# rhasspy/larynx

Hardware: AMD Instinct MI355X
Metric: utterances_per_sec (higher is better)
Workload: dtype f32; 1 GPU; en-us ljspeech GlowTTS + hifi_gan 'high', batch=1, 120 phoneme ids per utterance (~623 frames = 7.24 s audio), seeded random weights, device RNG noise, fused one-call entry (mi355tts_synthesize), denoiser off (the Python API default); ids_per_utterance=120, parallelism=utterance-dp1, batch=1, calls_in_flight_per_gpu=8

## Files before the change

### include/mi355tts.h

```cpp
#ifndef MI355TTS_H
#define MI355TTS_H

#include <stddef.h>
#include <stdint.h>

#ifdef __cplusplus
extern "C" {
#endif

#define MI355TTS_ABI_VERSION 2

typedef enum {
  MI355TTS_OK = 0,
  MI355TTS_ERR_INVALID = -1,
  MI355TTS_ERR_HIP = -2,
  MI355TTS_ERR_NOMEM = -3,
  MI355TTS_ERR_TOO_SMALL = -4,
  MI355TTS_ERR_NO_MODEL = -5
} mi355tts_status;

typedef struct mi355tts_ctx mi355tts_ctx;
typedef struct mi355tts_mel mi355tts_mel;

typedef struct {
// ... 157 lines not shown
  int32_t sample_rate, hop, window, tau_min, tau_max;
  float threshold;
  int32_t interpolate;
} mi355tts_pitch_params;
int mi355tts_load_pitch(mi355tts_ctx* ctx, const mi355tts_pitch_params* params, int* model_out);
int64_t mi355tts_pitch_frames(mi355tts_ctx* ctx, int model, int64_t samples);
int mi355tts_pitch(mi355tts_ctx* ctx, int model, const float* in_f32, const int16_t* in_i16, const int64_t* samples, int B,
                   int64_t in_ld, float* f0_out, float* periodicity_out, float* level_db_out, float* cmnd_out, int64_t out_ld,
                   uint32_t flags);

typedef struct {
  int32_t up, down, window;
  int32_t pitch, resampler;
} mi355tts_shift_params;
int mi355tts_load_shift(mi355tts_ctx* ctx, const mi355tts_shift_params* params, const float* window, int* model_out);
int64_t mi355tts_shift_length(mi355tts_ctx* ctx, int model, int64_t samples);
int mi355tts_shift(mi355tts_ctx* ctx, int model, const float* in_f32, const int16_t* in_i16, const int64_t* samples, int B,
                   int64_t in_ld, const int32_t* positions_in, float* out_f32, int16_t* out_i16, int64_t out_ld, int pcm_mode,
                   int32_t* positions_out, int64_t pos_ld, float* f0_out, int64_t f0_ld, int64_t* samples_out, uint32_t flags);

int mi355tts_synthesize(mi355tts_ctx* ctx, int glow, int vocoder, const int64_t* ids, const int32_t* id_lens, int B,
                        int ids_ld, float noise_scale, float length_scale, const float* noise, int noise_ld, uint64_t seed,
                        const mi355tts_audio_settings* audio, float denoiser_strength, int32_t pad_before,
                        int32_t pad_after, int32_t* frames_out, float* wav_f32, int16_t* wav_i16, int64_t wav_ld,
                        uint32_t flags);

int mi355tts_synthesize_speakers(mi355tts_ctx* ctx, int glow, int vocoder, const int64_t* ids, const int32_t* id_lens, int B,
                                 int ids_ld, float noise_scale, float length_scale, const float* noise, int noise_ld,
                                 uint64_t seed, const int32_t* speaker_ids, const mi355tts_audio_settings* audio,
                                 float denoiser_strength, int32_t pad_before, int32_t pad_after, int32_t* frames_out,
                                 float* wav_f32, int16_t* wav_i16, int64_t wav_ld, uint32_t flags);

int mi355tts_synthesize_prosody(mi355tts_ctx* ctx, int glow, int vocoder, const int64_t* ids, const int32_t* id_lens, int B,
                                int ids_ld, float noise_scale, float length_scale, const float* noise, int noise_ld,
                                uint64_t seed, const int32_t* speaker_ids, const mi355tts_audio_settings* audio,
                                float denoiser_strength, int32_t pad_before, int32_t pad_after, int32_t* frames_out,
                                float* wav_f32, int16_t* wav_i16, int64_t wav_ld, uint32_t flags,
                                const mi355tts_prosody* prosody);

int mi355tts_reserve(mi355tts_ctx* ctx, int workers, int glow, int vocoder, int max_batch, int max_ids, int max_frames,
                     int denoiser, int max_pad_samples);
int mi355tts_worker_queue_groups(mi355tts_ctx* ctx, int32_t* groups, int capacity);

int mi355tts_op_conv1d(mi355tts_ctx* ctx, const float* x, int B, int Cin, int L, const int32_t* lens, const float* w,
                       const float* bias, int Cout, int K, int dilation, float in_slope, int out_act, float* y);
int mi355tts_op_conv_transpose1d(mi355tts_ctx* ctx, const float* x, int B, int Cin, int L, const float* w,
                                 const float* bias, int Cout, int K, int stride, float in_slope, float* y);

int mi355tts_op_denoise(mi355tts_ctx* ctx, const float* wav, int B, int64_t N, const float* bias_spec, float strength,
                        float* out);

int mi355tts_op_gauss_noise(mi355tts_ctx* ctx, uint64_t seed, int B, int C, int T, float* out);

int mi355tts_op_maximum_path(mi355tts_ctx* ctx, const float* value, int B, int P_ld, int F_ld, const int32_t* id_lens,
                             const int32_t* frames, int32_t* durations_out, int dur_ld, float* score_out);

int mi355tts_hifigan_infer_taps(mi355tts_ctx* ctx, int vocoder, const mi355tts_mel* mel, float* wav_f32, int64_t wav_ld, char* json,
                                int cap);
int mi355tts_voc_tap_copy(mi355tts_ctx* ctx, int index, float* dst, int64_t cap);

int mi355tts_bench_conv1d(mi355tts_ctx* ctx, int B, int Cin, int Cout, int K, int dilation, int L, int tile_shape,
                          int iters, float* ms_per_launch);

int mi355tts_set_profiling(mi355tts_ctx* ctx, int enabled);
int mi355tts_set_option(mi355tts_ctx* ctx, const char* name, int value);
int mi355tts_call_coalesce_default(void);
int mi355tts_coalesce_stats(mi355tts_ctx* ctx, int64_t* passes, int64_t* rows);
int mi355tts_dispatch_selfcheck(mi355tts_ctx* ctx, int* state, float* plain_us, float* snake_us);
int mi355tts_profile_reset(mi355tts_ctx* ctx);
int mi355tts_profile_json(mi355tts_ctx* ctx, char* buf, int cap);
int mi355tts_profile_kernels_json(mi355tts_ctx* ctx, char* buf, int cap);
int mi355tts_kernel_counts_json(mi355tts_ctx* ctx, char* buf, int cap);
int mi355tts_profile_event_overhead(mi355tts_ctx* ctx, int pairs, double* us_out);

#ifdef __cplusplus
}
#endif
#endif
```

### larynx_amd/csrc/conv_mfma.h

```cpp
#pragma once
#include <hip/hip_runtime.h>
#include "prio.h"
#include "tile_grid.h"

#ifdef MI355TTS_ABLATION
#define MI355TTS_ABLATE(a, bit) ((a).ablate & (bit))
#else
#define MI355TTS_ABLATE(a, bit) 0
#endif

#ifndef CONV_STAMP
#define CONV_STAMP(n)
#endif
#ifndef CONV_WG_STAMP
#define CONV_WG_STAMP(lin, which)
#endif
#ifndef CONV_CHUNK_STAMP
#define CONV_CHUNK_STAMP(chunk, which)
#endif
#ifndef MI355TTS_ARING
#define MI355TTS_ARING 3
#endif

namespace mi355tts {


typedef float floatx16 __attribute__((ext_vector_type(16)));

enum ConvEpilogue {
  EPI_LINEAR = 0,
  EPI_GATE = 1,
  EPI_COUPLING = 2,
  EPI_UPSAMPLE = 3,
};

enum OutAct { ACT_NONE = 0, ACT_RELU = 1, ACT_TANH = 2 };

struct ConvArgs {
  const float* x;
  const float* x2;
  const float* x3;
  float in_div;
  long long x_bs;
  int x_ld;
  const int* in_len;
  int in_mul;
  int in_const;
  const float* w;
  const float* bias;
  int noct;
  int Cin;
  int rows;
  int dil;
  int pad;
  float in_slope;
  float* y;
  long long y_bs;
  int y_ld;
  const float* res;
  float* y2;
  long long y2_bs;
  int y2_ld;
  int split;
  int accum;
  int accum2;
  float alpha;
  int out_act;
  const int* out_len;
  int out_mul;
  int out_const;
  int up;
  int up_pad;
  int half;
  const float* cond;
  long long cond_bs;
  float* mix_x0;
  const float* mix_w;
  const float* mix_bias;
  const float* mix_scale;
  int ablate;
  int rows_major;
  const void* w16;
  int nslab;
};

template <int K, int EPI>
__device__ __forceinline__ int conv_n_len(const ConvArgs& a, int b) {
  if constexpr (EPI == EPI_UPSAMPLE) {
    const int Lin = a.in_len ? a.in_len[b] * a.in_mul : a.in_const;
    return Lin > 0 ? Lin + (K - 1) : 0;
  } else {
    return a.out_len ? a.out_len[b] * a.out_mul : a.out_const;
  }
}

template <int K, int CI_C, int MB, int NB, int WN, int KS, int HALO, int EPI, int WM = 1>
constexpr int conv_lds_floats() {
  constexpr bool SCATTER = (EPI == EPI_LINEAR || EPI == EPI_GATE);
  constexpr int NBR = (SCATTER && NB > 2) ? 1 : NB;
  constexpr int RED = (KS - 1) * WM * WN * NBR * 16 * 64;
  constexpr int XS = 2 * CI_C * (WN * NB * 32 + HALO);
  return XS > RED ? XS : RED;
}

template <int K, int CI_C, int MB, int NB, int WN, int KS, int HALO, int EPI, int WM = 1>
__device__ __forceinline__ void conv_tile(const ConvArgs& a, const int tile_x, const int tile_y, const int b, float* __restrict__ xs) {
  static_assert(WM == 1 || EPI == EPI_LINEAR || EPI == EPI_UPSAMPLE, "row groups of waves: linear and upsample epilogues");
  constexpr int NWAVES = WM * WN * KS;
  constexpr int WX = WM * WN;
  constexpr int NT = 64 * NWAVES;
  constexpr int T_T = WN * NB * 32;
  constexpr int XW = T_T + HALO;
  constexpr int OCTS = CI_C / 8;
  constexpr int NO = OCTS / KS;
  constexpr int S = NO * K;
  constexpr bool SCATTER = (EPI == EPI_LINEAR || EPI == EPI_GATE);
  constexpr int NBR = (SCATTER && NB > 2) ? 1 : NB;
  constexpr int RED = (KS - 1) * WX * NBR * 16 * 64;
  constexpr int LDSF = conv_lds_floats<K, CI_C, MB, NB, WN, KS, HALO, EPI, WM>();
  static_assert(CI_C % 8 == 0 && CI_C % NWAVES == 0 && OCTS % KS == 0, "bad tile parameters");

  const int tid = threadIdx.x;
  const int lane = tid & 63;
  const int wave = tid >> 6;
  const int wm = wave % WM;
  const int wn = (wave / WM) % WN;
  const int kg = wave / WX;
  const int wx = wm * WN + wn;
  const int t0 = tile_x * T_T;
  const int mt0 = (tile_y * WM + wm) * MB;

  const int Lin = a.in_len ? a.in_len[b] * a.in_mul : a.in_const;
  const int Lout = a.out_len ? a.out_len[b] * a.out_mul : a.out_const;
  const int n_len = (EPI == EPI_UPSAMPLE) ? (Lin > 0 ? Lin + (K - 1) : 0) : Lout;
  if (t0 >= n_len) return;

  const int roww = T_T + (K - 1) * a.dil;
  const float slope = a.in_slope;
  const float* xb = a.x + (long long)b * a.x_bs;
  const float* xb2 = a.x2 ? a.x2 + (long long)b * a.x_bs : nullptr;
  const float* xb3 = a.x3 ? a.x3 + (long long)b * a.x_bs : nullptr;
  const int nchunks = ((a.Cin + 7) / 8 + OCTS - 1) / OCTS;

  constexpr int XW4 = XW / 4;
  constexpr int NF4 = CI_C * XW4;
  constexpr int NE = (NF4 + NT - 1) / NT;
  static_assert(XW % 4 == 0, "LDS row stride must be a multiple of 4 floats");
  constexpr bool PD1 = (WN == 1 && KS == 8 && MB == 2 && K >= 7);
  float4 preA[NE], preB[PD1 ? 1 : NE];
  const int PA = (a.pad + 3) & ~3;
  const int used4 = (PA - a.pad + roww + 3) >> 2;
  const int cin_last = a.Cin - 1;
  const int ld_last4 = a.x_ld - 4;
  auto gload = [&](int chunk, float4 (&pre)[NE]) {
    int off[NE];
#pragma unroll
    for (int i = 0; i < NE; ++i) {
      const int e = tid + NT * i;
      const int row = e / XW4, f = e - row * XW4;
      const int ci = chunk * CI_C + (row < CI_C ? row : CI_C - 1);
      const int c0 = t0 - PA + 4 * f;
      off[i] = (ci < a.Cin ? ci : cin_last) * a.x_ld + (c0 < 0 ? 0 : (c0 > ld_last4 ? ld_last4 : c0));
    }
#pragma unroll
    for (int i = 0; i < NE; ++i) pre[i] = *reinterpret_cast<const float4*>(xb + off[i]);
#ifndef MI355TTS_PROBE_NO_X2
    if (xb2) {
      float4 t2[NE];
#pragma unroll
      for (int i = 0; i < NE; ++i) t2[i] = *reinterpret_cast<const float4*>(xb2 + off[i]);
#pragma unroll
      for (int i = 0; i < NE; ++i) {
        pre[i].x += t2[i].x;
        pre[i].y += t2[i].y;
        pre[i].z += t2[i].z;
        pre[i].w += t2[i].w;
      }
      if (xb3) {
#pragma unroll
        for (int i = 0; i < NE; ++i) t2[i] = *reinterpret_cast<const float4*>(xb3 + off[i]);
#pragma unroll
        for (int i = 0; i < NE; ++i) {
          pre[i].x += t2[i].x;
          pre[i].y += t2[i].y;
          pre[i].z += t2[i].z;
          pre[i].w += t2[i].w;
        }
      }
#pragma unroll
      for (int i = 0; i < NE; ++i) {
        pre[i].x = pre[i].x / a.in_div;
        pre[i].y = pre[i].y / a.in_div;
        pre[i].z = pre[i].z / a.in_div;
        pre[i].w = pre[i].w / a.in_div;
      }
    }
#endif
  };
  auto lstore = [&](int buf, int chunk, const float4 (&pre)[NE]) {
    float4* dst = reinterpret_cast<float4*>(xs + buf * (CI_C * XW));
#pragma unroll
    for (int i = 0; i < NE; ++i) {
      const int e = tid + NT * i;
      const int row = e / XW4, f = e - row * XW4;
      const int c0 = t0 - PA + 4 * f;
      const bool fok = chunk * CI_C + row < a.Cin && f < used4;
      float4 v = pre[i];
      v.x = (fok && c0 >= 0 && c0 < Lin) ? v.x : 0.f;
      v.y = (fok && c0 + 1 >= 0 && c0 + 1 < Lin) ? v.y : 0.f;
      v.z = (fok && c0 + 2 >= 0 && c0 + 2 < Lin) ? v.z : 0.f;
      v.w = (fok && c0 + 3 >= 0 && c0 + 3 < Lin) ? v.w : 0.f;
      v.x = v.x > 0.f ? v.x : v.x * slope;
      v.y = v.y > 0.f ? v.y : v.y * slope;
      v.z = v.z > 0.f ? v.z : v.z * slope;
      v.w = v.w > 0.f ? v.w : v.w * slope;
      if (e < NF4) dst[e] = v;
    }
  };

  floatx16 acc[MB][NB];
#pragma unroll
  for (int mb = 0; mb < MB; ++mb)
#pragma unroll
    for (int nb = 0; nb < NB; ++nb)
#pragma unroll
      for (int r = 0; r < 16; ++r) acc[mb][nb][r] = 0.f;

  const float4* wq[MB];
#pragma unroll
  for (int mb = 0; mb < MB; ++mb)
    wq[mb] = reinterpret_cast<const float4*>(a.w) + (long long)(mt0 + mb) * a.noct * K * 64 + lane;
  const int last_chunk = nchunks - 1;
  const int last_step = nchunks * S - 1;
  auto a_index = [&](int chunk, int q) -> long long {
    int g = chunk * S + q;
    g = g < last_step ? g : last_step;
    const int ch = g / S;
    q = g - ch * S;
    const int oi = q / K;
    const int k = q - oi * K;
    return (long long)(((ch * OCTS + kg + oi * KS) * K + k)) * 64;
  };

  constexpr int RD = MI355TTS_ARING;
  float4 ar[RD][MB];

  CONV_STAMP(0);
// ... 142 lines not shown
#pragma unroll
              for (int rr = 0; rr < R; ++rr)
                own[mb][nb0 + nbi][rr] += red[((((kg * (KS - 1) + si) * WX + wx) * NBR + nbi) * R + rr) * 64 + lane];
        }
    }
  } else if constexpr (KS > 1) {
    float* red = xs;
#pragma unroll
    for (int mb = 0; mb < MB; ++mb) {
      if (mb > 0) __syncthreads();
      if (kg > 0) {
#pragma unroll
        for (int nb = 0; nb < NB; ++nb)
#pragma unroll
          for (int r = 0; r < 16; ++r)
            red[((((kg - 1) * WX + wx) * NB + nb) * 16 + r) * 64 + lane] = acc[mb][nb][r];
      }
      __syncthreads();
      if (kg == 0) {
#pragma unroll
        for (int g = 1; g < KS; ++g)
#pragma unroll
          for (int nb = 0; nb < NB; ++nb)
#pragma unroll
            for (int r = 0; r < 16; ++r)
              acc[mb][nb][r] += red[((((g - 1) * WX + wx) * NB + nb) * 16 + r) * 64 + lane];
      }
    }
    if (kg > 0) return;
  }

  CONV_STAMP(4);
  const int col = lane & 31;
  const int rbase = 4 * (lane >> 5);

  if constexpr (EPI == EPI_LINEAR) {
    int rowin[R];
#pragma unroll
    for (int rr = 0; rr < R; ++rr) {
      const int r = kg * R + rr;
      rowin[rr] = acc_row(r) + rbase;
    }
#pragma unroll
    for (int mb = 0; mb < MB; ++mb) {
      const int row0 = (mt0 + mb) * 32;
      const bool first = row0 < a.split;
      float* yp = first ? a.y : a.y2;
      const long long ybs = first ? a.y_bs : a.y2_bs;
      const int yld = first ? a.y_ld : a.y2_ld;
      const int rowoff = first ? 0 : a.split;
      const float* rp = first ? a.res : nullptr;
      const bool acc_on = first ? (a.accum != 0) : (a.accum2 != 0);
      const float alpha = first ? a.alpha : 1.0f;
      const int act = first ? a.out_act : (int)ACT_NONE;
      float bb[R];
      int roff[R];
      bool rok[R];
#pragma unroll
      for (int rr = 0; rr < R; ++rr) {
        const int row = row0 + rowin[rr];
        bb[rr] = a.bias ? a.bias[row] : 0.f;
        rok[rr] = row < a.rows;
        roff[rr] = ((rok[rr] ? row : a.rows - 1) - rowoff) * yld;
      }
      float v[NB][R];
      int tcol[NB];
      bool tok[NB];
#pragma unroll
      for (int nb = 0; nb < NB; ++nb) {
        const int t = t0 + (wn * NB + nb) * 32 + col;
        tok[nb] = t < Lout;
        tcol[nb] = tok[nb] ? t : Lout - 1;
#pragma unroll
        for (int rr = 0; rr < R; ++rr) v[nb][rr] = own[mb][nb][rr] + bb[rr];
      }
      float* yb = yp + (long long)b * ybs;
      if (rp) {
        const float* rb = rp + (long long)b * ybs;
        float rv[NB][R];
#pragma unroll
        for (int nb = 0; nb < NB; ++nb)
#pragma unroll
          for (int rr = 0; rr < R; ++rr) rv[nb][rr] = rb[roff[rr] + tcol[nb]];
#pragma unroll
        for (int nb = 0; nb < NB; ++nb)
#pragma unroll
          for (int rr = 0; rr < R; ++rr) v[nb][rr] += rv[nb][rr];
      }
#pragma unroll
      for (int nb = 0; nb < NB; ++nb)
#pragma unroll
        for (int rr = 0; rr < R; ++rr) v[nb][rr] *= alpha;
      if (acc_on) {
        float ov[NB][R];
#pragma unroll
        for (int nb = 0; nb < NB; ++nb)
#pragma unroll
          for (int rr = 0; rr < R; ++rr) ov[nb][rr] = yb[roff[rr] + tcol[nb]];
#pragma unroll
        for (int nb = 0; nb < NB; ++nb)
#pragma unroll
          for (int rr = 0; rr < R; ++rr) v[nb][rr] += ov[nb][rr];
      }
      if (act == ACT_RELU) {
#pragma unroll
        for (int nb = 0; nb < NB; ++nb)
#pragma unroll
          for (int rr = 0; rr < R; ++rr) v[nb][rr] = v[nb][rr] > 0.f ? v[nb][rr] : 0.f;
      } else if (act == ACT_TANH) {
#pragma unroll
        for (int nb = 0; nb < NB; ++nb)
#pragma unroll
          for (int rr = 0; rr < R; ++rr) v[nb][rr] = tanhf(v[nb][rr]);
      }
#pragma unroll
      for (int nb = 0; nb < NB; ++nb)
#pragma unroll
        for (int rr = 0; rr < R; ++rr)
          if (rok[rr] && tok[nb]) yb[roff[rr] + tcol[nb]] = v[nb][rr];
    }
  } else if constexpr (EPI == EPI_GATE) {
    static_assert(MB == 1, "paired epilogues use one 32-row tile: 16 rows of each half");
    constexpr int H = R / 2;
    static_assert(H >= 1, "GATE needs at most 8 k-groups");
    float b0[H], b1[H];
    int off[H];
    bool cok[H];
#pragma unroll
    for (int rr = 0; rr < H; ++rr) {
      const int r = kg * H + rr;
      const int i = acc_row(r) + rbase;
      b0[rr] = a.bias ? a.bias[mt0 * 32 + i] : 0.f;
      b1[rr] = a.bias ? a.bias[mt0 * 32 + 16 + i] : 0.f;
      const int c = tile_y * 16 + i;
      cok[rr] = c < a.half;
      if (a.cond) {
        const float* cd = a.cond + (long long)b * a.cond_bs + (cok[rr] ? c : a.half - 1);
        b0[rr] += cd[0];
        b1[rr] += cd[a.half];
      }
      off[rr] = (cok[rr] ? c : a.half - 1) * a.y_ld;
    }
#pragma unroll
    for (int nb = 0; nb < NB; ++nb) {
      const int t = t0 + (wn * NB + nb) * 32 + col;
      const bool tok = t < Lout;
      float* yb = a.y + (long long)b * a.y_bs + (tok ? t : Lout - 1);
#pragma unroll
      for (int rr = 0; rr < H; ++rr) {
        const float v0 = own[0][nb][rr] + b0[rr];
        const float v1 = own[0][nb][H + rr] + b1[rr];
        const float out = tanhf(v0) * (1.0f / (1.0f + expf(-v1)));
        if (cok[rr] && tok) yb[off[rr]] = out;
      }
    }
  } else if constexpr (EPI == EPI_COUPLING) {
    static_assert(MB == 1, "paired epilogues use one 32-row tile: 16 rows of each half");
    float b0[8], b1[8];
#pragma unroll
    for (int r = 0; r < 8; ++r) {
      const int i = (r & 3) + 8 * (r >> 2) + rbase;
      b0[r] = a.bias ? a.bias[mt0 * 32 + i] : 0.f;
      b1[r] = a.bias ? a.bias[mt0 * 32 + 16 + i] : 0.f;
    }
#pragma unroll
    for (int nb = 0; nb < NB; ++nb) {
// ... 73 lines not shown
            const int row0 = (mt0 + mb) * 32 + 8 * g4 + rbase;
            if (row0 >= a.rows) continue;
            const int co = row0 / a.up;
            const int n0 = q * a.up + (row0 - co * a.up) - a.up_pad;
            float* dst = a.y + (long long)b * a.y_bs + (long long)co * a.y_ld + n0;
            if (n0 >= 0 && n0 + 3 < Lout) {
              *reinterpret_cast<float4*>(dst) = make_float4(acc[mb][nb][4 * g4] + bb[4 * g4], acc[mb][nb][4 * g4 + 1] + bb[4 * g4 + 1],
                                                            acc[mb][nb][4 * g4 + 2] + bb[4 * g4 + 2], acc[mb][nb][4 * g4 + 3] + bb[4 * g4 + 3]);
            } else {
#pragma unroll
              for (int e = 0; e < 4; ++e)
                if (n0 + e >= 0 && n0 + e < Lout) dst[e] = acc[mb][nb][4 * g4 + e] + bb[4 * g4 + e];
            }
          }
          continue;
        }
#ifndef MI355TTS_NO_UP2_PAIR
        if (a.up == 2) {
#pragma unroll
          for (int r = 0; r < 16; r += 2) {
            const int row = (mt0 + mb) * 32 + (r & 3) + 8 * (r >> 2) + rbase;
            if (row >= a.rows) continue;
            const int co = row >> 1;
            const int n0 = q * 2 - a.up_pad;
            float* dst = a.y + (long long)b * a.y_bs + (long long)co * a.y_ld + n0;
            const float v0 = acc[mb][nb][r] + bb[r], v1 = acc[mb][nb][r + 1] + bb[r + 1];
            if (n0 >= 0 && n0 + 1 < Lout && row + 1 < a.rows) {
              typedef float up_float2 __attribute__((ext_vector_type(2), aligned(4)));
              *reinterpret_cast<up_float2*>(dst) = up_float2{v0, v1};
            } else {
              if (n0 >= 0 && n0 < Lout) dst[0] = v0;
              if (row + 1 < a.rows && n0 + 1 >= 0 && n0 + 1 < Lout) dst[1] = v1;
            }
          }
          continue;
        }
#endif
#pragma unroll
        for (int r = 0; r < 16; ++r) {
          const int row = (mt0 + mb) * 32 + (r & 3) + 8 * (r >> 2) + rbase;
          if (row >= a.rows) continue;
          const int co = row / a.up;
          const int ph = row - co * a.up;
          const int n = q * a.up + ph - a.up_pad;
          if (n < 0 || n >= Lout) continue;
          a.y[(long long)b * a.y_bs + (long long)co * a.y_ld + n] = acc[mb][nb][r] + bb[r];
        }
      }
    }
  }
}


template <int K, int CI_C, int MB, int NB, int WN, int KS, int HALO, int EPI, int WM = 1>
__global__ __launch_bounds__(64 * WM * WN * KS, ((EPI == EPI_LINEAR && ((NB == 1 && MB == 2) || (MB == 1 && NB == 2 && KS == 4))) || WM == 4) ? 4 : 1) void conv_mfma_kernel(const ConvArgs a) {
  __shared__ float xs[conv_lds_floats<K, CI_C, MB, NB, WN, KS, HALO, EPI, WM>()];
  int tile_x, tile_y;
  int gx = gridDim.x;
  const int lin = blockIdx.x + blockIdx.y * gridDim.x;
  if (gridDim.z > 1) {
    gx = row_tiles(conv_n_len<K, EPI>(a, blockIdx.z), WN * NB * 32);
    if (lin >= gx * (int)gridDim.y) return;
  }
  xcd_tile_lin(lin, gx, gridDim.y, tile_x, tile_y, a.rows_major);
  conv_tile<K, CI_C, MB, NB, WN, KS, HALO, EPI, WM>(a, tile_x, tile_y, blockIdx.z, xs);
  CONV_STAMP(5);
}

constexpr int GROUP_MAX_SEG = 8;
struct ConvGroupArgs {
  ConvArgs c[3];
  int gx[3], gy[3];
  int off[4];
  int nseg = 0;
  int seg_off[GROUP_MAX_SEG + 1];
  int seg_first[GROUP_MAX_SEG];
  int seg_m[GROUP_MAX_SEG];
};

inline void group_snake_order(ConvGroupArgs& g, int ncu, int slots) {
  g.nseg = 0;
  const int total = g.off[3];
  if (ncu <= 0 || (ncu & 7) || total <= ncu || total > slots) return;
  struct Piece { int m, first, n; };
  Piece out[GROUP_MAX_SEG];
  int nout = 0;
  for (int r0 = 0; r0 < total; r0 += ncu) {
    const int r1 = r0 + ncu < total ? r0 + ncu : total;
    Piece round[3];
    int nr = 0;
    for (int m = 0; m < 3; ++m) {
      const int a = g.off[m] > r0 ? g.off[m] : r0, b = g.off[m + 1] < r1 ? g.off[m + 1] : r1;
      if (b > a) round[nr++] = Piece{m, a - g.off[m], b - a};
    }
    const bool rev = ((r0 / ncu) & 1) != 0;
    for (int i = 0; i < nr; ++i) {
      const Piece& pc = round[rev ? nr - 1 - i : i];
      if (nout && out[nout - 1].m == pc.m && out[nout - 1].first + out[nout - 1].n == pc.first) {
        out[nout - 1].n += pc.n;
        continue;
      }
      if (nout == GROUP_MAX_SEG) return;
      out[nout++] = pc;
    }
  }
  int o = 0;
  for (int i = 0; i < nout; ++i) {
    g.seg_off[i] = o;
    g.seg_first[i] = out[i].first;
    g.seg_m[i] = out[i].m;
    o += out[i].n;
  }
  g.seg_off[nout] = o;
  g.nseg = nout;
}

inline double group_order_imbalance(const ConvGroupArgs& g, int ncu, const int real[3], const double cost[3]) {
  if (ncu <= 0 || ncu > 4096) return 1e9;
// ... 54 lines not shown
```

### larynx_amd/csrc/hifigan_forward.h

```cpp
#pragma once

extern "C" int mi355tts_hifigan_hop(mi355tts_ctx* ctx, int vocoder) {
  if (!ctx) return fail(MI355TTS_ERR_INVALID, "ctx null");
  std::shared_ptr<HifiModel> vpin;
  CHECK(find_model(ctx, vocoder, &vpin));
  return vpin->hop;
}

struct VocCall {
  float denoiser_strength = 0.f;
  float* wav_f32 = nullptr;
  int16_t* wav_i16 = nullptr;
  int64_t wav_ld = 0;
  uint32_t flags = 0;
  int pad_before = 0, pad_after = 0;
  const VocRow* rows = nullptr;
  int precision = -1;
  VocTaps* taps = nullptr;
};

static int ensure_denoiser_bias(mi355tts_ctx* ctx, HifiModel* hm, int vocoder, int precision);

static int hifigan_precheck(mi355tts_ctx* ctx, HifiModel* hm, int vocoder, const int32_t* frames, int B, int M, int Fmax, VocCall& c) {
  if (c.precision < 0) c.precision = hm->precision.load();
// ... 90 lines not shown
  VocTaps* taps;

  VocPass(CallFrame& f, HifiModel* hm_, const mi355tts_mel* mel_, const VocCall& call)
      : frame(f), ctx(f.ctx), w(f.w), hm(hm_), mel(mel_), s(f.s), B(mel_->B), F(mel_->max_frames), hop(hm_->hop), d_frames(mel_->frames_dev),
        voc_host_len(mel_->B == 1 ? mel_->frames[0] : -1), opt(f.w->opt), prec(call.precision), f16(call.precision == MI355TTS_PRECISION_F16),
        denoiser_strength(call.denoiser_strength), denoise(call.denoiser_strength > 0.f && mel_->max_frames > 0),
        out_dev((call.flags & MI355TTS_OUT_DEVICE) != 0), taps(call.taps) {}

  RowLen rows(int mul) const { return row_len(B, voc_host_len, d_frames, mul); }
  template <class P>
  P* plane(int i) const { return reinterpret_cast<P*>(buf[i]); }

  int bind(const VocCall& call, const OutRows& out) {
    const mi355tts_hifigan_hparams& h = hm->hp;
    if (f16 && !hm->f16_ok) return fail(MI355TTS_ERR_INVALID, "internal: fp16 mode on a vocoder it does not cover");
    bias_spec = hm->bias_spec[f16 ? 1 : 0];
    if (denoise && !bias_spec) return fail(MI355TTS_ERR_INVALID, "internal: no denoiser bias for this precision");
    voc_out = f16 || (!opt.env.voc_out_off && opt.voc_out && hm->post_C == (h.upsample_initial_channel >> h.num_upsamples) && hm->post.K == 7);
    if (call.rows && !voc_out) return fail(MI355TTS_ERR_INVALID, "internal: per-row outputs need the voc_out tail");
    for (int b = 0; b < B; ++b) {
      const OutRow r = out(b);
      pads = std::max(pads, (int)(r.pad_before + r.pad_after));
      any_f32 = any_f32 || r.f32;
      any_i16 = any_i16 || r.i16;
    }
    const HifiLayout lay = hifi_layout(h, hop, B, F, denoise, f16 || hifi_split_out(opt.serial_branches, h), pads);
    if (f16 && (size_t)((mel->M + 7) / 8) * F * 16 > lay.plane * sizeof(float)) return fail(MI355TTS_ERR_INVALID, "internal: mel octets exceed a plane buffer");
    staged = host_staging(B, any_f32 && !out_dev, (size_t)F * hop, any_i16 && !out_dev, (size_t)F * hop + (size_t)pads);
    CHECK(frame.reserve(lay.total, staged.end()));
    char* base = w->arena;
    for (int i = 0; i < lay.nbuf; ++i) buf[i] = (float*)(base + lay.o_buf[i]);
    wav = (float*)(base + lay.o_wav);
    wav2 = (float*)(base + lay.o_wav2);
    fbuf = (float*)(base + lay.o_fbuf);
    i16 = (short*)(base + lay.o_i16);
    peaks = (unsigned*)(base + lay.o_peak);
    Nld = lay.Nld;
    ild = Nld + (size_t)pads;
    Tmax = lay.Tmax;
    peak_ld = (long long)(Nld / POST_TW + 2);
    peak = voc_out && any_i16 && !denoise ? reinterpret_cast<float*>(peaks) : nullptr;
    return 0;
  }
};

static std::string tap_name(const char* fmt, ...) {
  char tmp[64];
  va_list ap;
  va_start(ap, fmt);
  std::vsnprintf(tmp, sizeof(tmp), fmt, ap);
  va_end(ap);
  return tmp;
}
static int voc_tap(VocPass& p, const std::string& name, const void* x, bool f16, int ch, int ld, int mul) {
  VocTaps& T = *p.taps;
  VocTap t;
  t.name = name;
  t.kn = T.last_kn;
  t.f16 = f16;
  t.B = p.B;
  t.ch = ch;
  t.ld = ld;
  for (int b = 0; b < p.B; ++b) t.len.push_back((int)std::min<long long>((long long)p.mel->frames[b] * mul, ld));
  t.bytes = f16 ? (size_t)p.B * (size_t)((ch + 7) / 8) * (size_t)ld * 16 : sizeof(float) * (size_t)p.B * (size_t)ch * (size_t)ld;
  if (T.bytes + t.bytes > VocTaps::MAX_BYTES)
    return fail(MI355TTS_ERR_NOMEM, "the planes of this call exceed %zu MB of tap copies (at '%s'): fewer frames or rows", VocTaps::MAX_BYTES >> 20, name.c_str());
  HIPCHECK(hipMalloc(&t.dev, t.bytes));
  T.bytes += t.bytes;
  T.taps.push_back(t);
  HIPCHECK(hipMemcpyAsync(t.dev, x, t.bytes, hipMemcpyDeviceToDevice, p.s));
  return 0;
}

struct VocStage {
  int i, u, ku, cout, Lout, ldo, mul;
  long long bs;
};
static VocStage voc_stage(const mi355tts_hifigan_hparams& h, int i, int Lin, int mul, bool f16) {
  VocStage st;
  st.i = i;
  st.u = h.upsample_rates[i];
  st.ku = h.upsample_kernel_sizes[i];
  st.cout = h.upsample_initial_channel >> (i + 1);
  st.Lout = Lin * st.u;
  st.ldo = f16 ? st.Lout : (st.Lout + 3) & ~3;
  st.mul = mul * st.u;
  st.bs = f16 ? (long long)(st.cout / 8) * st.ldo : (long long)st.cout * st.ldo;
  return st;
}

template <class P>
struct StageCursor {
  P* cur[3] = {nullptr, nullptr, nullptr};
  int ncur = 1;
  float div = 1.0f;
  int ch = 0, Lin = 0, ldin = 0, mul = 1;
  int flip = 0;

  template <class Args>
  void inputs(Args& a) const {
    a.x = cur[0];
    if (ncur > 1) {
      a.x2 = cur[1];
      a.x3 = ncur > 2 ? cur[2] : nullptr;
      a.in_div = div;
    }
  }
  void advance(const VocStage& st, P* const* outs, int n, float d, bool flipped) {
    for (int j = 0; j < 3; ++j) cur[j] = j < n ? outs[j] : nullptr;
    ncur = n;
    div = d;
    ch = st.cout;
// ... 24 lines not shown
  if (n_side > 0) {
    HIPCHECK(hipEventRecord(w->ev_fork, s));
    for (int j = 0; j < n_side; ++j) HIPCHECK(hipStreamWaitEvent(w->aux[j], w->ev_fork, 0));
  }
  CHECK(body());
  for (int j = 0; j < n_side; ++j) {
    HIPCHECK(hipEventRecord(w->ev_join[j], w->aux[j]));
    HIPCHECK(hipStreamWaitEvent(s, w->ev_join[j], 0));
  }
  return 0;
}

struct F32Schedule {
  bool split_out, grouped, concurrent;
  int rb_tiles;
};
static int f32_schedule(const VocPass& p, F32Schedule& sc) {
  const mi355tts_hifigan_hparams& h = p.hm->hp;
  const CallOptions& opt = p.opt;
  Worker* w = p.w;
  sc.split_out = hifi_split_out(opt.serial_branches, h);
  const bool busy = opt.adaptive_schedule && p.ctx->active_calls.load(std::memory_order_relaxed) > 1;
  sc.grouped = sc.split_out && h.num_kernels == 3 && opt.mrf_group && !busy;
  sc.concurrent = sc.split_out && !opt.mrf_group && !busy;
  if (p.taps && sc.concurrent)
    return fail(MI355TTS_ERR_INVALID, "taps: the forked schedule (\"mrf_group\" = 0) runs its chains on side streams a copy cannot be ordered behind");
  if (sc.concurrent && !w->aux[0]) {
    for (int i = 0; i < 2; ++i) {
      HIPCHECK(hipStreamCreateWithFlags(&w->aux[i], hipStreamNonBlocking));
      HIPCHECK(hipEventCreateWithFlags(&w->ev_join[i], hipEventDisableTiming));
    }
    HIPCHECK(hipEventCreateWithFlags(&w->ev_fork, hipEventDisableTiming));
  }
  sc.rb_tiles = opt.env.rb_tiles > 0 ? opt.env.rb_tiles : 1024;
  return 0;
}

static int f32_pre(VocPass& p, StageCursor<float>& c) {
  const int C0 = p.hm->hp.upsample_initial_channel, Fp = (p.F + 3) & ~3;
  c.cur[0] = p.buf[0];
  c.ch = C0;
  c.Lin = p.F;
  c.ldin = Fp;
  ConvArgs a = base_args(p.mel->voc, (long long)p.mel->M * p.mel->ld, p.mel->ld, p.d_frames, 1, c.cur[0], (long long)C0 * Fp, Fp, p.d_frames, 1, 1, 3);
  if (p.taps) CHECK(voc_tap(p, "mel", p.mel->voc, false, p.mel->M, p.mel->ld, 1));
  CHECK(launch_conv(p.ctx, p.w, p.hm->pre, a, EPI_LINEAR, p.B, p.F, KC_VOC_IO, nullptr, 1024, p.voc_host_len));
  if (p.taps) CHECK(voc_tap(p, "pre", c.cur[0], false, C0, Fp, 1));
  return 0;
}

static int f32_upsample(VocPass& p, const StageCursor<float>& c, const VocStage& st) {
  ConvArgs a = base_args(c.cur[0], (long long)c.ch * c.ldin, c.ldin, p.d_frames, c.mul, p.buf[1], st.bs, st.ldo, p.d_frames, st.mul, 1, st.ku / st.u - 1);
  c.inputs(a);
  a.in_slope = 0.1f;
  a.up = st.u;
  a.up_pad = (st.ku - st.u) / 2;
  CHECK(launch_conv(p.ctx, p.w, p.hm->ups[st.i], a, EPI_UPSAMPLE, p.B, c.Lin + st.ku / st.u - 1, KC_UPSAMPLE, nullptr, 1024, p.voc_host_len, p.prec));
  if (p.taps) CHECK(voc_tap(p, tap_name("up%d", st.i), p.buf[1], false, st.cout, st.ldo, st.mul));
  return 0;
}

struct VocStep {
  PairPlan pair;
  ConvPlan c1, c2;
  float* dst;
};
static int run_step_grouped(mi355tts_ctx* ctx, Worker* w, const VocStep (&sp)[3], hipStream_t s) {
  const int npair = sp[0].pair.ok + sp[1].pair.ok + sp[2].pair.ok;
  if (npair == 3) {
    const PairPlan* pairs[3] = {&sp[0].pair, &sp[1].pair, &sp[2].pair};
    return run_pair_group(ctx, w, pairs, 3, s);
  }
  if (npair != 0) return 1;
  const ConvPlan* c1[3] = {&sp[0].c1, &sp[1].c1, &sp[2].c1};
  const ConvPlan* c2[3] = {&sp[0].c2, &sp[1].c2, &sp[2].c2};
  const int rc = run_group(ctx, w, c1, 3, s);
  if (rc != 0 || sp[0].c2.empty) return rc;
  const int rc2 = run_group(ctx, w, c2, 3, s);
  if (rc2 == 1)
    for (int j = 0; j < 3; ++j) CHECK(run_plan(ctx, w, sp[j].c2, s));
  return rc2 < 0 ? rc2 : 0;
}

struct F32Chains {
  VocPass& p;
  const F32Schedule& sc;
  const VocStage& st;
  int nk, nd;
  ChainPlanes<float> pl[MI355TTS_MAX_STAGES];
  const float* rin[MI355TTS_MAX_STAGES];
  hipStream_t stream[MI355TTS_MAX_STAGES];

  F32Chains(VocPass& p_, const F32Schedule& sc_, const VocStage& st_, int flip)
      : p(p_), sc(sc_), st(st_), nk(p_.hm->hp.num_kernels), nd(p_.hm->hp.num_dilations) {
    for (int j = 0; j < nk; ++j) {
      pl[j] = chain_planes<float>(p, j, flip, sc.split_out);
      rin[j] = p.buf[1];
      stream[j] = (sc.concurrent && j > 0) ? p.w->aux[j - 1] : p.s;
    }
  }

  int plan_step(int j, int d, VocStep& sp) const {
    const mi355tts_hifigan_hparams& h = p.hm->hp;
    const HifiResConv& rc = p.hm->rb[st.i][j][d];
    const int kk = h.resblock_kernel_sizes[j], B = p.B, ldo = st.ldo, mul = st.mul, Lout = st.Lout, host_len = p.voc_host_len;
    const long long bs = st.bs;
    const int* d_frames = p.d_frames;
    const float* x = rin[j];
    const float inv_nk = 1.0f / (float)nk;
    sp.dst = step_dst(pl[j], d, nd);
    if (!sp.dst) return fail(MI355TTS_ERR_INVALID, "internal: resblock scratch aliasing");
    const bool fold = d == nd - 1 && !sc.split_out;
    sp.pair.ok = false;
    if (h.resblock_type == 1) {
      plan_pair(p.opt, rc.c1, rc.c2, x, sp.dst, bs, ldo, d_frames, mul, rc.dil, fold ? inv_nk : 1.0f, fold ? (j > 0) : 0, B, Lout, host_len,
                &sp.pair, p.prec);
      if (sp.pair.ok) return 0;
      ConvArgs a = base_args(x, bs, ldo, d_frames, mul, pl[j].t, bs, ldo, d_frames, mul, rc.dil, (kk * rc.dil - rc.dil) / 2);
      a.in_slope = 0.1f;
      CHECK(plan_conv(p.opt, rc.c1, a, EPI_LINEAR, B, Lout, KC_RESBLOCK, sc.rb_tiles, host_len, &sp.c1, p.prec));
      ConvArgs c2 = base_args(pl[j].t, bs, ldo, d_frames, mul, sp.dst, bs, ldo, d_frames, mul, 1, (kk - 1) / 2);
      c2.in_slope = 0.1f;
      c2.res = x;
      if (fold) {
        c2.alpha = inv_nk;
        c2.accum = j > 0;
      }
      CHECK(plan_conv(p.opt, rc.c2, c2, EPI_LINEAR, B, Lout, KC_RESBLOCK, sc.rb_tiles, host_len, &sp.c2, p.prec));
    } else {
      ConvArgs a = base_args(x, bs, ldo, d_frames, mul, sp.dst, bs, ldo, d_frames, mul, rc.dil, (kk * rc.dil - rc.dil) / 2);
      a.in_slope = 0.1f;
      a.res = x;
      if (fold) {
        a.alpha = inv_nk;
        a.accum = j > 0;
      }
      CHECK(plan_conv(p.opt, rc.c1, a, EPI_LINEAR, B, Lout, KC_RESBLOCK, sc.rb_tiles, host_len, &sp.c1, p.prec));
      sp.c2.empty = true;
    }
    return 0;
  }
  int tap_step(int j, int d, const VocStep& sp) const {
    const bool fold = d == nd - 1 && !sc.split_out;
    if (!sp.pair.ok && !sp.c2.empty) CHECK(voc_tap(p, tap_name("rb%d.%d.%d.t", st.i, j, d), pl[j].t, false, st.cout, st.ldo, st.mul));
    if (!fold) return voc_tap(p, tap_name("rb%d.%d.%d", st.i, j, d), sp.dst, false, st.cout, st.ldo, st.mul);
    return j == nk - 1 ? voc_tap(p, tap_name("stage%d", st.i), sp.dst, false, st.cout, st.ldo, st.mul) : 0;
  }
  int run_step_alone(int j, const VocStep& sp) const {
    if (sp.pair.ok) return run_pair(p.ctx, p.w, sp.pair, stream[j]);
    CHECK(run_plan(p.ctx, p.w, sp.c1, stream[j]));
    return run_plan(p.ctx, p.w, sp.c2, stream[j]);
  }
  int run_dilation_major() {
    for (int d = 0; d < nd; ++d) {
      VocStep sp[3];
      for (int j = 0; j < nk; ++j) CHECK(plan_step(j, d, sp[j]));
      if (nk == 3 && !sp[0].pair.ok && !sp[1].pair.ok && !sp[2].pair.ok) {
        ConvPlan* c1s[3] = {&sp[0].c1, &sp[1].c1, &sp[2].c1};
        ConvPlan* c2s[3] = {&sp[0].c2, &sp[1].c2, &sp[2].c2};
        promote_group_plans(p.opt, c1s, nk);
        promote_group_plans(p.opt, c2s, nk);
      }
      const int rc = sc.grouped ? run_step_grouped(p.ctx, p.w, sp, p.s) : 1;
      if (rc < 0) return rc;
      if (rc == 1)
        for (int j = 0; j < nk; ++j) CHECK(run_step_alone(j, sp[j]));
      if (p.taps)
        for (int j = 0; j < nk; ++j) CHECK(tap_step(j, d, sp[j]));
      for (int j = 0; j < nk; ++j) rin[j] = sp[j].dst;
    }
    return 0;
  }
  int run_chain_major() {
    for (int j = 0; j < nk; ++j)
      for (int d = 0; d < nd; ++d) {
        VocStep sp;
        CHECK(plan_step(j, d, sp));
        CHECK(run_step_alone(j, sp));
        if (p.taps) CHECK(tap_step(j, d, sp));
        rin[j] = sp.dst;
      }
    return 0;
  }
};

static int f32_resblocks(VocPass& p, const F32Schedule& sc, StageCursor<float>& c, const VocStage& st) {
  HifiModel* hm = p.hm;
  const int nk = hm->hp.num_kernels;
  if (p.opt.mrf_small && !p.opt.serial_branches && st.i < (int)hm->mrf.size() && hm->mrf[st.i].ok) {
    float* sums[2] = {p.buf[0], p.buf[2]};
    CHECK(run_mrf_small(p.ctx, p.w, hm->mrf[st.i], hm->arena, p.buf[1], sums[0], sums[1], st.bs, st.ldo, p.d_frames, st.mul, p.B, st.Lout, p.voc_host_len, p.s));
    if (p.taps)
      for (int m = 0; m < 2; ++m) CHECK(voc_tap(p, tap_name("stage%d.sum%d", st.i, m), sums[m], false, st.cout, st.ldo, st.mul));
    c.advance(st, sums, 2, (float)nk, false);
    return 0;
  }
  F32Chains chains(p, sc, st, c.flip);
  CHECK(run_forked(p.w, p.s, sc.concurrent ? nk - 1 : 0, [&] { return sc.split_out ? chains.run_dilation_major() : chains.run_chain_major(); }));
  if (sc.split_out) {
    float* outs[3] = {nullptr, nullptr, nullptr};
    for (int j = 0; j < nk; ++j) outs[j] = chains.pl[j].dst_last;
    c.advance(st, outs, nk, (float)nk, true);
  } else {
    std::swap(p.buf[5], p.buf[0]);
    c.advance(st, &p.buf[0], 1, 1.0f, false);
  }
  return 0;
}

template <class Args, class P>
static Args post_args(const VocPass& p, const StageCursor<P>& c, long long x_bs) {
  Args a;
  std::memset(&a, 0, sizeof(a));
  a.in_div = 1.0f;
  c.inputs(a);
  a.slope = 0.01f;
  a.x_bs = x_bs;
  a.x_ld = c.ldin;
  p.rows(c.mul).into(a);
  a.len_mul = c.mul;
  a.w = p.hm->arena + p.hm->post_w_off;
  a.bias = p.hm->arena + p.hm->post_b_off;
  a.C = c.ch;
  a.y = p.wav;
  a.y_bs = (long long)p.Nld;
  return a;
}

static int f32_post(VocPass& p, const StageCursor<float>& c) {
  if (!p.voc_out) {
    ConvArgs a = base_args(c.cur[0], (long long)c.ch * c.ldin, c.ldin, p.d_frames, c.mul, p.wav, (long long)p.Nld, (int)p.Nld, p.d_frames, c.mul, 1, 3);
    c.inputs(a);
    a.in_slope = 0.01f;
    a.out_act = ACT_TANH;
    CHECK(launch_conv(p.ctx, p.w, p.hm->post, a, EPI_LINEAR, p.B, c.Lin, KC_VOC_IO, nullptr, 1024, p.voc_host_len));
    if (p.taps) CHECK(voc_tap(p, "wav", p.wav, false, 1, (int)p.Nld, c.mul));
    return 0;
  }
  PostArgs a = post_args<PostArgs>(p, c, (long long)c.ch * c.ldin);
  if (p.peak) {
    a.peak = p.peak;
    a.peak_ld = p.peak_ld;
  }
  {
    ProfScope ps(p.ctx, p.w, KC_VOC_IO, 2.0 * (double)c.ch * 7 * (double)c.Lin * p.B);
    ps.kernel(KN_POST_CONV);
    const dim3 pg((c.Lin + POST_TW - 1) / POST_TW, p.B);
    switch_const<1, 2, 3>(c.ncur, [&](auto n) { hipLaunchKernelGGL(HIP_KERNEL_NAME(post_conv_kernel<7, decltype(n)::value>), pg, dim3(256), 0, p.s, a); });
  }
  if (p.taps) CHECK(voc_tap(p, "wav", p.wav, false, 1, (int)p.Nld, c.mul));
  return 0;
}

static int hifigan_body_f32(VocPass& p) {
  F32Schedule sc;
  CHECK(f32_schedule(p, sc));
  StageCursor<float> c;
  CHECK(f32_pre(p, c));
  for (int i = 0; i < p.hm->hp.num_upsamples; ++i) {
    const VocStage st = voc_stage(p.hm->hp, i, c.Lin, c.mul, false);
    CHECK(f32_upsample(p, c, st));
    CHECK(f32_resblocks(p, sc, c, st));
  }
  return f32_post(p, c);
}

struct HPlane {
  uint4* x;
  int ch, ld, mul;
};
static HConvArgs f16_conv_args(const VocPass& p, const HPlane& in, const HPlane& out, int dil, int pad) {
  HConvArgs a;
  std::memset(&a, 0, sizeof(a));
  a.x = in.x;
  a.x_bs = (long long)(in.ch / 8) * in.ld;
  a.x_ld = in.ld;
  a.in_div = 1.0f;
  a.dil = dil;
  a.pad = pad;
  a.in_slope = 1.0f;
  a.out_slope = 1.0f;
  a.y = out.x;
  a.y_bs = (long long)(out.ch / 8) * out.ld;
  a.y_ld = out.ld;
  a.cout = out.ch;
  h_set_lengths(a, p.B, p.d_frames, p.voc_host_len, in.mul, out.mul);
  return a;
}

static int f16_pre(VocPass& p, StageCursor<uint4>& c) {
  const mi355tts_mel* mel = p.mel;
  const int B = p.B, F = p.F, M = mel->M, moct = (M + 7) / 8, C0 = p.hm->hp.upsample_initial_channel;
  uint4* melh = p.plane<uint4>(1);
  {
    ProfScope ps(p.ctx, p.w, KC_SMALL, 0, p.s);
    ps.kernel(KN_PACK_OCTETS);
    hipLaunchKernelGGL(pack_octets_kernel, dim3((F + 255) / 256, moct, B), dim3(256), 0, p.s, mel->voc, (long long)mel->M * mel->ld, mel->ld, M, p.d_frames, 1,
                       melh, (long long)moct * F, F);
  }
  if (p.taps) CHECK(voc_tap(p, "mel", melh, true, 8 * moct, F, 1));
  c.cur[0] = p.plane<uint4>(0);
// ... 43 lines not shown
static int f16_resblocks(VocPass& p, StageCursor<uint4>& c, const VocStage& st) {
  const mi355tts_hifigan_hparams& h = p.hm->hp;
  const int nk = h.num_kernels, nd = h.num_dilations, B = p.B, ch = st.cout, Lout = st.Lout;
  ChainPlanes<uint4> pl[3];
  uint4* rin[3];
  auto plane = [&](uint4* x) { return HPlane{x, ch, st.ldo, st.mul}; };
  for (int j = 0; j < nk; ++j) {
    pl[j] = chain_planes<uint4>(p, j, c.flip, true);
    rin[j] = p.plane<uint4>(1);
  }
  const bool use_group = p.opt.mrf_group, use_pair = h.resblock_type == 1 && use_group && p.opt.rb_pair;
  for (int d = 0; d < nd; ++d) {
    HPlan c1[3], c2[3];
    HPairPlan pp[3];
    uint4* dst[3];
    for (int j = 0; j < nk; ++j) {
      const HResConv& rc = p.hm->h_rb[st.i][j][d];
      const int K = h.resblock_kernel_sizes[j], dil = h.resblock_dilations[j][d];
      const double flop = 2.0 * ch * ch * K * (double)Lout * B;
      dst[j] = step_dst(pl[j], d, nd);
      if (h.resblock_type == 1) {
        HConvArgs a1 = f16_conv_args(p, plane(rin[j]), plane(pl[j].t), dil, (K * dil - dil) / 2);
        HConvArgs a2 = f16_conv_args(p, plane(pl[j].t), plane(dst[j]), 1, (K - 1) / 2);
        a1.in_slope = a1.out_slope = 0.1f;
        a2.res = rin[j];
        c1[j] = plan_f16(rc.c1, a1, EPI_LINEAR, B, Lout, flop);
        c2[j] = plan_f16(rc.c2, a2, EPI_LINEAR, B, Lout, flop);
        pp[j].a = f16_pair_args(p, st, rc, rin[j], dst[j], dil);
        pp[j].K = K;
        pp[j].flop = 2.0 * flop;
      } else {
        HConvArgs a = f16_conv_args(p, plane(rin[j]), plane(dst[j]), dil, (K * dil - dil) / 2);
        a.in_slope = 0.1f;
        a.res = rin[j];
        c1[j] = plan_f16(rc.c1, a, EPI_LINEAR, B, Lout, flop);
      }
    }
    int fused = 1;
    if (use_pair) {
      fused = run_pair_group_f16(p.ctx, p.w, pp, nk, ch, B, Lout, p.s);
      if (fused < 0) return fused;
      if (fused == 0 && p.taps)
        for (int j = 0; j < nk; ++j) CHECK(voc_tap(p, tap_name("rb%d.%d.%d", st.i, j, d), dst[j], true, ch, st.ldo, st.mul));
    }
    for (int pass = 0; fused != 0 && pass < (h.resblock_type == 1 ? 2 : 1); ++pass) {
      const HPlan* plans = pass ? c2 : c1;
      int rc = use_group ? run_group_f16(p.ctx, p.w, plans, nk, B, p.s) : 1;
      if (rc < 0) return rc;
      if (rc == 1)
        for (int j = 0; j < nk; ++j) CHECK(run_plan_f16(p.ctx, p.w, plans[j], KC_RESBLOCK, p.s));
      if (p.taps) {
        const bool t_plane = h.resblock_type == 1 && pass == 0;
        for (int j = 0; j < nk; ++j)
          CHECK(voc_tap(p, tap_name(t_plane ? "rb%d.%d.%d.t" : "rb%d.%d.%d", st.i, j, d), t_plane ? pl[j].t : dst[j], true, ch, st.ldo, st.mul));
      }
    }
    for (int j = 0; j < nk; ++j) rin[j] = dst[j];
  }
  uint4* outs[3] = {nullptr, nullptr, nullptr};
  for (int j = 0; j < nk; ++j) outs[j] = pl[j].dst_last;
  c.advance(st, outs, nk, (float)nk, true);
  return 0;
}

static int f16_post(VocPass& p, const StageCursor<uint4>& c) {
  HPostArgs a = post_args<HPostArgs>(p, c, (long long)(c.ch / 8) * c.ldin);
  a.peak = p.peak;
  a.peak_ld = p.peak_ld;
  {
    ProfScope ps(p.ctx, p.w, KC_VOC_IO, 2.0 * (double)c.ch * 7 * (double)c.Lin * p.B, p.s);
    ps.kernel(KN_POST_F16);
    const dim3 pg((c.Lin + HPOST_TW - 1) / HPOST_TW, p.B);
    switch_const<1, 2, 3>(c.ncur, [&](auto n) { hipLaunchKernelGGL(HIP_KERNEL_NAME(post_f16_kernel<7, decltype(n)::value>), pg, dim3(256), 0, p.s, a); });
  }
  if (p.taps) CHECK(voc_tap(p, "wav", p.wav, false, 1, (int)p.Nld, c.mul));
  return 0;
}

static int hifigan_body_f16(VocPass& p) {
  StageCursor<uint4> c;
  CHECK(f16_pre(p, c));
  for (int i = 0; i < p.hm->hp.num_upsamples; ++i) {
    const VocStage st = voc_stage(p.hm->hp, i, c.Lin, c.mul, true);
    CHECK(f16_upsample(p, c, st));
    CHECK(f16_resblocks(p, c, st));
  }
  return f16_post(p, c);
}

static float* voc_denoise(VocPass& p) {
  if (!p.denoise) return p.wav;
  ProfScope ps(p.ctx, p.w, KC_SMALL, 0);
  hipLaunchKernelGGL(stft_denoise_kernel, dim3(p.Tmax, p.B), dim3(256), 0, p.s, p.wav, (long long)p.Nld, p.d_frames, p.hop, p.bias_spec,
                     p.denoiser_strength, p.fbuf, p.Tmax, (float*)nullptr);
  hipLaunchKernelGGL(overlap_add_kernel, dim3(256, p.B), dim3(256), 0, p.s, p.fbuf, p.Tmax, p.d_frames, p.hop, p.wav2, (long long)p.Nld,
                     (long long)p.Nld);
  return p.wav2;
}

static int voc_tail_one_launch(VocPass& p, const VocCall& call, float* wav) {
  const bool out_dev = p.out_dev;
  const int B = p.B;
  ProfScope ps(p.ctx, p.w, KC_SMALL, 0);
  if (p.any_i16 && !p.peak) {
    HIPCHECK(hipMemsetAsync(p.peaks, 0, sizeof(unsigned) * B, p.s));
    hipLaunchKernelGGL(absmax_kernel, dim3(128, B), dim3(256), 0, p.s, wav, (long long)p.Nld, p.d_frames, p.hop, p.peaks);
  }
// ... 105 lines not shown
    c.flags = MI355TTS_OUT_DEVICE;
    c.precision = precision;
    rc = hifigan_call_on(ctx, hm, vocoder, zm, c);
  }
  if (!rc) {
    CallFrame f(ctx);
    rc = f.open();
    if (!rc) {
      hipLaunchKernelGGL(stft_denoise_kernel, dim3(1, 1), dim3(256), 0, f.s, dwav, (long long)N, zm->frames_dev, hop,
                         (const float*)nullptr, 0.f, (float*)nullptr, 1, bias);
      if (f.wait() != hipSuccess) rc = fail(MI355TTS_ERR_HIP, "denoiser bias kernel failed");
    }
  }
  mel_destroy(zm);
  if (dwav) hipFree(dwav);
  if (rc) {
    if (bias) hipFree(bias);
    return rc;
  }
  hm->bias_spec[bi] = bias;
  hm->bias_ready[bi] = true;
  return 0;
}

static int hifigan_call(mi355tts_ctx* ctx, int vocoder, const mi355tts_mel* mel, const VocCall& call) {
  if (!ctx || !mel) return fail(MI355TTS_ERR_INVALID, "null argument");
  std::shared_ptr<HifiModel> vpin;
  CHECK(find_model(ctx, vocoder, &vpin));
  return hifigan_call_on(ctx, vpin.get(), vocoder, mel, call);
}

extern "C" int mi355tts_hifigan_infer_padded(mi355tts_ctx* ctx, int vocoder, const mi355tts_mel* mel, float denoiser_strength,
                                             float* wav_f32, int16_t* wav_i16, int64_t wav_ld, uint32_t flags,
                                             int32_t pad_before, int32_t pad_after) {
  VocCall c;
  c.denoiser_strength = denoiser_strength;
  c.wav_f32 = wav_f32;
  c.wav_i16 = wav_i16;
  c.wav_ld = wav_ld;
  c.flags = flags;
  c.pad_before = pad_before;
  c.pad_after = pad_after;
  return hifigan_call(ctx, vocoder, mel, c);
}

static std::string voc_taps_json(const VocTaps& T) {
  std::string s = "[";
  for (size_t i = 0; i < T.taps.size(); ++i) {
    const VocTap& t = T.taps[i];
    char tmp[256];
    std::snprintf(tmp, sizeof(tmp), "%s{\"name\": \"%s\", \"channels\": %d, \"ld\": %d, \"len\": [", i ? ", " : "", t.name.c_str(), t.ch, t.ld);
    s += tmp;
    for (size_t b = 0; b < t.len.size(); ++b) s += (b ? ", " : "") + std::to_string(t.len[b]);
    std::snprintf(tmp, sizeof(tmp), "], \"f16\": %d, \"kernel\": \"%s\"}", t.f16 ? 1 : 0, t.kn >= 0 && t.kn < KN_COUNT ? kname_name[t.kn] : "-");
    s += tmp;
  }
  return s + "]";
}

extern "C" int mi355tts_hifigan_infer_taps(mi355tts_ctx* ctx, int vocoder, const mi355tts_mel* mel, float* wav_f32, int64_t wav_ld,
                                           char* json, int cap) {
  if (!ctx || !mel || !wav_f32 || !json) return fail(MI355TTS_ERR_INVALID, "null argument");
  auto taps = std::make_shared<VocTaps>();
  VocCall c;
  c.wav_f32 = wav_f32;
  c.wav_ld = wav_ld;
  c.taps = taps.get();
  CHECK(hifigan_call(ctx, vocoder, mel, c));
  const std::string s = voc_taps_json(*taps);
  {
    std::lock_guard<std::mutex> lk(ctx->mu);
    ctx->voc_taps = taps;
  }
  return copy_json(s, json, cap, "tap list buffer too small");
}

extern "C" int mi355tts_voc_tap_copy(mi355tts_ctx* ctx, int index, float* dst, int64_t cap) {
  if (!ctx || !dst) return fail(MI355TTS_ERR_INVALID, "null argument");
  std::shared_ptr<VocTaps> taps;
  {
    std::lock_guard<std::mutex> lk(ctx->mu);
    taps = ctx->voc_taps;
  }
  if (!taps || index < 0 || (size_t)index >= taps->taps.size()) return fail(MI355TTS_ERR_INVALID, "no tap %d (mi355tts_hifigan_infer_taps first)", index);
  const VocTap& t = taps->taps[(size_t)index];
  const size_t n = (size_t)t.B * t.ch * t.ld;
  if ((size_t)std::max<int64_t>(cap, 0) < n) return fail(MI355TTS_ERR_TOO_SMALL, "tap %d holds %zu floats", index, n);
  HIPCHECK(hipSetDevice(ctx->device));
  if (!t.f16) {
    HIPCHECK(hipMemcpy(dst, t.dev, t.bytes, hipMemcpyDeviceToHost));
    return 0;
  }
  std::vector<_Float16> h(t.bytes / sizeof(_Float16));
  HIPCHECK(hipMemcpy(h.data(), t.dev, t.bytes, hipMemcpyDeviceToHost));
  const size_t noct = (size_t)t.ch / 8, ld = (size_t)t.ld;
  for (size_t b = 0; b < (size_t)t.B; ++b)
    for (size_t o = 0; o < noct; ++o)
      for (size_t col = 0; col < ld; ++col)
        for (size_t e = 0; e < 8; ++e) dst[(b * t.ch + 8 * o + e) * ld + col] = (float)h[((b * noct + o) * ld + col) * 8 + e];
  return 0;
}

extern "C" int mi355tts_hifigan_infer(mi355tts_ctx* ctx, int vocoder, const mi355tts_mel* mel, float denoiser_strength,
                                      float* wav_f32, int16_t* wav_i16, int64_t wav_ld, uint32_t flags) {
  return mi355tts_hifigan_infer_padded(ctx, vocoder, mel, denoiser_strength, wav_f32, wav_i16, wav_ld, flags, 0, 0);
}
```

### larynx_amd/csrc/host_context.h

```cpp
#pragma once

#include "host_profile.h"

static hipError_t mi355_sync(hipStream_t s) {
  const int mode = g_sync_mode.load(std::memory_order_relaxed);
  if (mode == 1) {
    constexpr int MAXDEV = 16;
    thread_local hipEvent_t evs[MAXDEV] = {};
    int dev = 0;
    if (hipGetDevice(&dev) != hipSuccess || dev < 0 || dev >= MAXDEV) return hipStreamSynchronize(s);
    if (!evs[dev] && hipEventCreateWithFlags(&evs[dev], hipEventBlockingSync | hipEventDisableTiming) != hipSuccess) {
      evs[dev] = nullptr;
      return hipStreamSynchronize(s);
    }
    hipError_t e = hipEventRecord(evs[dev], s);
    return e == hipSuccess ? hipEventSynchronize(evs[dev]) : e;
  }
  if (mode == 2) {
    for (;;) {
      const hipError_t e = hipStreamQuery(s);
      if (e != hipErrorNotReady) return e;
      struct timespec ts = {0, 20000};
      nanosleep(&ts, nullptr);
    }
  }
  if (mode == 3) {
    struct timespec t0;
    clock_gettime(CLOCK_MONOTONIC, &t0);
    for (;;) {
      const hipError_t e = hipStreamQuery(s);
      if (e != hipErrorNotReady) return e;
      struct timespec t1;
      clock_gettime(CLOCK_MONOTONIC, &t1);
      if ((t1.tv_sec - t0.tv_sec) * 1000000000LL + (t1.tv_nsec - t0.tv_nsec) > 60000) break;
    }
    const int slack = prctl(PR_GET_TIMERSLACK, 0, 0, 0, 0);
    const bool lowered = slack > 1000 && prctl(PR_SET_TIMERSLACK, 1000UL, 0, 0, 0) == 0;
    hipError_t e;
    for (;;) {
      e = hipStreamQuery(s);
      if (e != hipErrorNotReady) break;
      struct timespec ts = {0, 20000};
      nanosleep(&ts, nullptr);
    }
    if (lowered) prctl(PR_SET_TIMERSLACK, (unsigned long)slack, 0, 0, 0);
    return e;
  }
  return hipStreamSynchronize(s);
}

struct Worker : ProfLane {
  char* arena = nullptr;
  size_t arena_bytes = 0;
  size_t arena_pos = 0;
  int* pinned = nullptr;
  size_t pinned_ints = 0;
  char* pinned_out = nullptr;
  size_t pinned_out_bytes = 0;
  int qgroup = -1;
  hipStream_t aux[2] = {nullptr, nullptr};
  hipEvent_t ev_fork = nullptr;
  hipEvent_t ev_join[2] = {nullptr, nullptr};
  CallOptions opt;
};

struct VocTap {
  std::string name;
  int kn = -1;
  bool f16 = false;
  int B = 0, ch = 0, ld = 0;
  std::vector<int> len;
  void* dev = nullptr;
  size_t bytes = 0;
};
struct VocTaps {
  static constexpr size_t MAX_BYTES = (size_t)256 << 20;
  std::vector<VocTap> taps;
  size_t bytes = 0;
  int last_kn = -1;
  VocTaps() = default;
  VocTaps(const VocTaps&) = delete;
  ~VocTaps() {
    for (auto& t : taps)
      if (t.dev) hipFree(t.dev);
  }
};

struct mi355tts_ctx : ProfSums {
  std::shared_ptr<VocTaps> voc_taps;
  int device = 0;
  int ncu = 256;
  std::mutex mu;
  struct ModelEntry {
    const char* kind;
    std::shared_ptr<void> model;
  };
  std::map<int, ModelEntry> models;
  float* gl_table = nullptr;
  float* hann_periodic = nullptr;
  int next_id = 1;
  std::vector<Worker*> free_workers;
  std::vector<Worker*> all_workers;
  ContextOptions opts;
  std::atomic<int> active_calls{0};
  std::vector<int> qgroup_busy;
  std::atomic<int> selfcheck_state{0};
  float selfcheck_plain_us = 0.f, selfcheck_snake_us = 0.f;
  std::mutex join_mu;
  std::condition_variable join_cv;
  std::vector<struct CallReq*> join_q;
  int join_inflight = 0, join_rows_inflight = 0;
  bool join_gathering = false;
  long long join_arrivals = 0;
  long long join_passes = 0, join_rows = 0;
  std::vector<std::pair<void*, size_t>> mel_pool;
  size_t mel_pool_cap = 256;
  std::map<void*, size_t> mel_sizes;
};

struct mi355tts_mel {
  mi355tts_ctx* ctx;
  int B, M, ld;
// ... 107 lines not shown
```

### larynx_amd/csrc/host_launch.h

```cpp
#pragma once

struct RowLen {
  const int* len;
  int len_const;
  template <class Args>
  void into(Args& a) const { a.len = len; a.len_const = len_const; }
};
static inline RowLen row_len(int B, int host_len, const int* dev_len, int mul = 1, int dev_const = 0) {
  if (B == 1 && host_len >= 0) return {nullptr, host_len * mul};
  return {dev_len, dev_const};
}

template <int K, int CI_C, int MB, int NB, int WN, int KS, int HALO, int EPI>
static void launch_conv_inst(ProfScope& ps, hipStream_t s, dim3 grid, const ConvArgs& a) {
  ps.kernel(KN_CONV_MFMA, a.rows);
  hipLaunchKernelGGL(HIP_KERNEL_NAME(conv_mfma_kernel<K, CI_C, MB, NB, WN, KS, HALO, EPI>), grid, dim3(64 * WN * KS), 0, s, a);
}

enum TileShape { TILE_SMALL = 0, TILE_W128 = 1, TILE_NB2 = 2, TILE_TINY = 3, TILE_LAST = 3, TILE_M128 = 4 };

static bool rb_plane_ok(const ConvArgs& a) { return (long long)a.Cin * a.x_ld < (1LL << 30); }

template <int K, int EPI>
static int launch_conv_k(ProfScope& ps, hipStream_t s, int MB, int shape, dim3 grid, const ConvArgs& a, bool rb_conv) {
  constexpr int HALO = conv_halo(K);
  constexpr int CI_SMALL = (K == 1) ? 64 : 32;
  constexpr bool PAIRED = (EPI == EPI_GATE || EPI == EPI_COUPLING);
  if (!halo_fits(K, a.dil, a.pad, HALO))
    return fail(MI355TTS_ERR_INVALID, "conv K=%d dilation=%d exceeds the staged halo", K, a.dil);
  if (a.x_ld % 4) return fail(MI355TTS_ERR_INVALID, "internal: activation row stride %d is not a multiple of 4", a.x_ld);
  if constexpr (EPI == EPI_LINEAR && K >= 3) {
    if (shape == TILE_M128) {
      ps.kernel(KN_CONV_M128, a.rows);
      hipLaunchKernelGGL(HIP_KERNEL_NAME(conv_mfma_kernel<K, 16, 1, 2, 1, 1, HALO, EPI, 4>), grid, dim3(256), 0, s, a);
      return 0;
    }
  }
  if constexpr (EPI == EPI_UPSAMPLE) {
    if (shape == TILE_M128) {
      if constexpr (K == 2) {
        if (rb_conv && a.Cin % 16 == 0 && !a.res && !a.accum && a.alpha == 1.0f && rb_plane_ok(a)) {
          if (a.x2 && a.x3) hipLaunchKernelGGL(HIP_KERNEL_NAME(rb_conv_kernel<2, 4, EPI_UPSAMPLE, true>), grid, dim3(256), 0, s, a);
          else if (!a.x2) hipLaunchKernelGGL(HIP_KERNEL_NAME(rb_conv_kernel<2, 4, EPI_UPSAMPLE, false>), grid, dim3(256), 0, s, a);
          if ((a.x2 && a.x3) || !a.x2) {
            ps.kernel(KN_RB_CONV, a.rows);
            return 0;
          }
        }
      }
      ps.kernel(KN_CONV_M128, a.rows);
      hipLaunchKernelGGL(HIP_KERNEL_NAME(conv_mfma_kernel<K, 16, 1, 2, 1, 1, HALO, EPI, 4>), grid, dim3(256), 0, s, a);
      return 0;
    }
  }
  if (shape == TILE_M128) return fail(MI355TTS_ERR_INVALID, "internal: the 128-row tile is a ResBlock conv / upsampler shape");
  if (MB == 1) {
    if (shape == TILE_TINY) launch_conv_inst<K, 64, 1, 1, 1, 8, HALO, EPI>(ps, s, grid, a);
    else if (shape == TILE_SMALL) launch_conv_inst<K, CI_SMALL, 1, 1, 2, 4, HALO, EPI>(ps, s, grid, a);
    else if (shape == TILE_W128) launch_conv_inst<K, 32, 1, 2, 2, 4, HALO, EPI>(ps, s, grid, a);
    else launch_conv_inst<K, 16, 1, 2, 4, 2, HALO, EPI>(ps, s, grid, a);
    return 0;
  }
  if constexpr (!PAIRED) {
    if (shape == TILE_TINY) launch_conv_inst<K, 64, 2, 1, 1, 8, HALO, EPI>(ps, s, grid, a);
    else if (shape == TILE_SMALL) launch_conv_inst<K, CI_SMALL, 2, 1, 2, 4, HALO, EPI>(ps, s, grid, a);
    else if (shape == TILE_W128) return fail(MI355TTS_ERR_INVALID, "internal: the 128-column tile is one m-tile high");
    else launch_conv_inst<K, 16, 2, 2, 4, 2, HALO, EPI>(ps, s, grid, a);
    return 0;
  }
  return fail(MI355TTS_ERR_INVALID, "paired epilogues run on 32-row tiles (MB == 1)");
}

struct ConvPlan {
  ConvArgs a;
  int K = 0, MB = 1, shape = TILE_TINY, epi = EPI_LINEAR, cls = 0;
  dim3 grid;
  double flop = 0;
  bool empty = true;
  int bf16 = 0;
  int n_max = 0;
  bool pinned = false;
};

enum Bf16Cfg {
  BF_A = 0,
  BF_B = 1,
  BF_C = 2,
  BF_D = 3,
  BF_K = 4,
};
struct Bf16Tile {
  int NB, WM, WN, KS;
};
constexpr Bf16Tile BF16_TILES[5] = {{4, 4, 1, 1}, {1, 4, 1, 1}, {2, 2, 2, 1}, {1, 1, 4, 1}, {4, 4, 1, 2}};
template <class F>
static bool bf16_dispatch(int cfg, int bf16, F&& f) {
  return switch_const<BF_A, BF_B, BF_C, BF_D, BF_K>(cfg, [&](auto c) {
    if (bf16 == 3) f(c, int_c<3>{});
    else f(c, int_c<1>{});
  });
}
template <int K, int EPI>
static int launch_bf16_k(int cfg, int bf16, dim3 grid, hipStream_t s, const ConvArgs& a) {
  const bool known = bf16_dispatch(cfg, bf16, [&](auto c, auto terms) {
// ... 132 lines not shown
  return rc;
}
static int run_plan(mi355tts_ctx* ctx, Worker* w, const ConvPlan& p, hipStream_t stream = nullptr) {
  if (p.empty) return 0;
  hipStream_t s = stream ? stream : w->stream;
  ProfScope ps(ctx, w, p.cls, p.flop, s);
  const bool rb_conv = w->opt.rb_conv && !w->opt.env.rb_conv_off;
  if (p.bf16) {
    ps.kernel(KN_CONV_BF16, p.a.rows);
    if (p.epi == EPI_UPSAMPLE) {
      if (p.K != 2) return fail(MI355TTS_ERR_INVALID, "bf16 upsampler needs two taps");
      return launch_bf16_k<2, EPI_UPSAMPLE>(p.shape, p.bf16, p.grid, s, p.a);
    }
    int rc = 0;
    if (!switch_const<3, 5, 7, 11>(p.K, [&](auto k) { rc = launch_bf16_k<decltype(k)::value, EPI_LINEAR>(p.shape, p.bf16, p.grid, s, p.a); }))
      rc = fail(MI355TTS_ERR_INVALID, "unsupported conv kernel size %d in bf16 mode", p.K);
    return rc;
  }
  if (p.epi == EPI_LINEAR) return launch_conv_taps<EPI_LINEAR, 1, 3, 5, 7, 11>(ps, p, "unsupported conv kernel size %d", s, rb_conv);
  if (p.epi == EPI_GATE) return launch_conv_taps<EPI_GATE, 3, 5>(ps, p, "unsupported WaveNet kernel size %d", s, rb_conv);
  if (p.epi == EPI_COUPLING) return launch_conv_taps<EPI_COUPLING, 1>(ps, p, "coupling conv must be 1x1", s, rb_conv);
  return launch_conv_taps<EPI_UPSAMPLE, 1, 2, 3>(ps, p, "unsupported upsample taps %d", s, rb_conv);
}

static int launch_conv(mi355tts_ctx* ctx, Worker* w, const DevConv& c, ConvArgs a, int epi, int B, int n_max, int cls,
                       hipStream_t stream = nullptr, int min_tiles = 1024, int host_len = -1, int precision = 0) {
  ConvPlan p;
  CHECK(plan_conv(w->opt, c, a, epi, B, n_max, cls, min_tiles, host_len, &p, precision));
  return run_plan(ctx, w, p, stream);
}

struct GroupTile {
  int shape, MB, CI_C, MBT, NB, WN, KS, WM;
};
constexpr GroupTile GROUP_TILES[6] = {{TILE_M128, 0, 16, 1, 2, 1, 1, 4}, {TILE_NB2, 2, 16, 2, 2, 4, 2, 1},  {TILE_W128, 1, 32, 1, 2, 2, 4, 1},
                                      {TILE_SMALL, 2, 32, 2, 1, 2, 4, 1}, {TILE_TINY, 1, 64, 1, 1, 1, 8, 1}, {TILE_TINY, 2, 64, 2, 1, 1, 8, 1}};
static int group_tile(int shape, int MB) {
  for (int i = 0; i < 6; ++i)
    if (GROUP_TILES[i].shape == shape && (GROUP_TILES[i].MB == MB || GROUP_TILES[i].MB == 0)) return i;
  return -1;
}
template <int K0, int K1, int K2>
static void launch_group_k(ProfScope& ps, hipStream_t s, int tile, dim3 grid, const ConvGroupArgs& g) {
  ps.kernel(KN_CONV_GROUP, g.c[0].rows);
  switch_const<0, 1, 2, 3, 4, 5>(tile, [&](auto i) {
    constexpr GroupTile t = GROUP_TILES[decltype(i)::value];
    hipLaunchKernelGGL(HIP_KERNEL_NAME(conv_group_kernel<K0, K1, K2, t.CI_C, t.MBT, t.NB, t.WN, t.KS, conv_halo(K0), conv_halo(K1), conv_halo(K2), t.WM>),
                       grid, dim3(64 * t.WM * t.WN * t.KS), 0, s, g);
  });
}
static bool rb_member_ok(const ConvArgs& a, int K) {
  const int halo = K == 11 ? RbCfg<11>::HALO : K == 7 ? RbCfg<7>::HALO : RbCfg<3>::HALO;
  return !a.x2 && !a.x3 && a.bias && a.alpha == 1.0f && !a.accum && a.out_act == ACT_NONE && a.split >= a.rows && !a.y2 &&
         a.rows % 128 == 0 && halo_fits(K, a.dil, a.pad, halo) && rb_plane_ok(a);
}

static void promote_group_plans(const CallOptions& o, ConvPlan* const* plans, int n) {
  if (n != 3 || o.env.group_promote_off || !o.group_promote) return;
  int K[3], tiles[3];
  for (int i = 0; i < 3; ++i) {
    const ConvPlan& p = *plans[i];
    if (p.empty || p.bf16 || p.pinned || p.epi != EPI_LINEAR || p.cls != KC_RESBLOCK || p.shape == TILE_M128 || p.grid.z != 1 ||
        p.n_max <= 0 || (p.a.x_ld % 4) || (p.K != 11 && p.K != 7 && p.K != 3) || !rb_member_ok(p.a, p.K))
      return;
    K[i] = p.K;
    tiles[i] = ((p.n_max + 63) / 64) * (p.a.rows / 128);
  }
  const GroupLayout lay = group_layout(K, tiles);
  const int ncu = o.ncu, total = lay.off[3];
  if (!lay.k1173 || total <= ncu) return;
  if (total <= 4 * ncu) {
    const double max_imbalance = o.env.promote_max_imbalance;
    ConvGroupArgs g;
    std::copy(lay.off, lay.off + 4, g.off);
    group_snake_order(g, ncu, 4 * ncu);
    const int real[3] = {tiles[lay.ord[0]], tiles[lay.ord[1]], tiles[lay.ord[2]]};
    const double cost[3] = {11.0, 7.0, 3.0};
    if (group_order_imbalance(g, ncu, real, cost) > max_imbalance) return;
  }
  for (int i = 0; i < 3; ++i) {
    ConvPlan& p = *plans[i];
    p.shape = TILE_M128;
    p.MB = 1;
    p.a.rows_major = 0;
    p.grid = dim3((p.n_max + 63) / 64, p.a.rows / 128, 1);
  }
}

template <int NB>
static void launch_rb_group(int dil, dim3 grid, hipStream_t s, const ConvGroupArgs& g) {
  const bool fixed = switch_const<1, 3, 5>(dil, [&](auto d) {
    hipLaunchKernelGGL(HIP_KERNEL_NAME(rb_group_dil_kernel<11, 7, 3, NB, decltype(d)::value>), grid, dim3(256), 0, s, g);
  });
  if (!fixed) hipLaunchKernelGGL(HIP_KERNEL_NAME(rb_group_kernel<11, 7, 3, NB>), grid, dim3(256), 0, s, g);
}

static int run_group(mi355tts_ctx* ctx, Worker* w, const ConvPlan* const* plans, int n, hipStream_t s) {
  const CallOptions& o = w->opt;
  if (o.env.group_off || n != 3) return 1;
  const int K[3] = {plans[0]->K, plans[1]->K, plans[2]->K};
  int tiles[3];
  for (int i = 0; i < 3; ++i) tiles[i] = (int)(plans[i]->grid.x * plans[i]->grid.y);
  const GroupLayout lay = group_layout(K, tiles);
  const int ncu = o.ncu;
  const ConvPlan* m[3] = {plans[lay.ord[0]], plans[lay.ord[1]], plans[lay.ord[2]]};
  const ConvPlan& p0 = *m[0];
  ConvGroupArgs g;
  double flop = 0;
  for (int i = 0; i < 3; ++i) {
    const ConvPlan& p = *m[i];
    if (p.empty || p.epi != EPI_LINEAR || p.shape != p0.shape || p.MB != p0.MB || p.grid.z != p0.grid.z || p.bf16 != p0.bf16) return 1;
    if (!halo_fits(p.K, p.a.dil, p.a.pad, conv_halo(p.K))) return 1;
    if (p.a.x_ld % 4) return 1;
    g.c[i] = p.a;
    g.gx[i] = (int)p.grid.x;
    g.gy[i] = (int)p.grid.y;
    flop += p.flop;
  }
  std::copy(lay.off, lay.off + 4, g.off);
  const dim3 grid(g.off[3], 1, p0.grid.z);
  const bool taps_ok = lay.k1173 || lay.k753;
  if (p0.bf16) {
    if (!taps_ok) return 1;
    ProfScope ps(ctx, w, p0.cls, flop, s);
    ps.kernel(KN_CONV_BF16_GROUP, p0.a.rows);
    bool known = false;
    switch_taps(lay, [&](auto k0, auto k1, auto k2) {
      constexpr int K0 = decltype(k0)::value, K1 = decltype(k1)::value, K2 = decltype(k2)::value;
      known = bf16_dispatch(p0.shape, p0.bf16, [&](auto c, auto terms) {
        constexpr Bf16Tile t = BF16_TILES[decltype(c)::value];
        hipLaunchKernelGGL(HIP_KERNEL_NAME(conv_bf16_group_kernel<K0, K1, K2, 1, t.NB, t.WM, t.WN, conv_halo(K0), conv_halo(K1), conv_halo(K2),
                                                                  decltype(terms)::value, t.KS>),
                           grid, dim3(64 * t.WM * t.WN * t.KS), 0, s, g);
      });
    });
    return known ? 0 : fail(MI355TTS_ERR_INVALID, "internal: bf16 tile %d", p0.shape);
  }
  const int tile = group_tile(p0.shape, p0.MB);
  if (tile < 0 || !taps_ok) return 1;
  ProfScope ps(ctx, w, p0.cls, flop, s);
  if (p0.shape == TILE_M128 && lay.k1173 && !o.env.rb_conv_off && o.rb_conv) {
    bool rb_ok = true;
    for (int i = 0; i < 3; ++i) rb_ok = rb_ok && rb_member_ok(g.c[i], i == 0 ? 11 : i == 1 ? 7 : 3);
    if (rb_ok) {
      const bool snake = o.group_snake && !o.env.snake_off;
      const int dil = (o.rb_dil && g.c[0].dil == g.c[1].dil && g.c[0].dil == g.c[2].dil) ? g.c[0].dil : 0;
      const int nb4_min = o.env.rb_nb4_min_tiles != KNOB_UNSET ? o.env.rb_nb4_min_tiles : (ctx->active_calls.load(std::memory_order_relaxed) > 1 ? 3 * ncu : 0);
      if (nb4_min > 0 && grid.z == 1) {
        int gx4[3], tiles4[3];
        for (int i = 0; i < 3; ++i) tiles4[i] = (gx4[i] = (m[i]->n_max + 127) / 128) * g.gy[i];
        if (tiles4[0] + tiles4[1] + tiles4[2] >= nb4_min) {
          std::copy(gx4, gx4 + 3, g.gx);
          group_offsets(tiles4, g.off);
          const dim3 grid4(g.off[3], 1, 1);
          if (snake) group_snake_order(g, ncu, 3 * ncu);
          ps.kernel(KN_RB_GROUP_NB4, p0.a.rows);
          launch_rb_group<4>(dil, grid4, s, g);
          return 0;
        }
      }
      if (grid.z == 1 && snake) group_snake_order(g, ncu, 4 * ncu);
      ps.kernel(g.nseg ? KN_RB_GROUP_SNAKE : KN_RB_GROUP, p0.a.rows);
      launch_rb_group<2>(dil, grid, s, g);
      return 0;
    }
  }
  switch_taps(lay, [&](auto k0, auto k1, auto k2) {
    launch_group_k<decltype(k0)::value, decltype(k1)::value, decltype(k2)::value>(ps, s, tile, grid, g);
  });
  return 0;
}

struct PairTile {
  int CB, NB, WN16, NB16;
};
constexpr PairTile PAIR_TILES[2] = {{1, 2, 4, 2}, {2, 1, 4, 2}};
template <class F>
static void pair_tile_dispatch(int C, F&& f) {
  if (C == 32) f(int_c<0>{});
  else f(int_c<1>{});
}
struct PairPlan {
  PairArgs a;
  int K = 0, C = 0, NB = 1;
  dim3 grid;
  double flop = 0;
  bool ok = false;
  int bf16 = 0;
  bool rb = false;
};
static void plan_pair(const CallOptions& o, const DevConv& c1, const DevConv& c2, const float* x, float* y, long long bs, int ld, const int* len,
                      int len_mul, int dil, float alpha, int accum, int B, int Lmax, int host_len, PairPlan* out, int precision = 0) {
  const int nb64 = 1;
  const int C = c1.Cout, K = c1.K;
  out->ok = false;
  const bool half = precision != MI355TTS_PRECISION_F32 && c1.w16 && c2.w16;
  if (half) {
    if (o.env.bf16_pair_off || c1.nslab16 != C / 16 || c2.nslab16 != C / 16 || c1.mtiles16 != C / 32 || c2.mtiles16 != C / 32) return;
  }
  if (o.env.pair_fusion_off || (C != 32 && C != 64) || c1.Cin != C || c2.Cin != C || c2.Cout != C || c2.K != K || dil > PAIR_DMAX || dil < 1 ||
      (K != 3 && K != 7 && K != 11) || c1.noct != c2.noct || !c1.has_bias || !c2.has_bias || (ld % 4) || x == y || Lmax <= 0)
    return;
  PairArgs& a = out->a;
  a.x = x;
  a.y = y;
  a.bs = bs;
  a.ld = ld;
  row_len(B, host_len, len, len_mul).into(a);
  a.len_mul = len_mul;
  a.w1 = c1.w;
  a.b1 = c1.bias;
  a.w2 = c2.w;
  a.b2 = c2.bias;
  a.noct = c1.noct;
  a.C = C;
  a.dil = dil;
// ... 170 lines not shown
  if (o.env.lin16_off || !o.glow_fuse || !c.l16_J || n_max <= 0 || (c.K == 1 && o.env.lin16_no_k1)) return 1;
  const int PA = (a.pad + 3) & ~3;
  if ((PA - a.pad) + (c.K - 1) * a.dil > MI355TTS_G16_HALO || a.x_ld % 4 || a.in_mul != a.out_mul || a.in_len != a.out_len) return 1;
  if (a.x2 || a.alpha != 1.0f || a.accum || a.in_slope != 1.0f || (a.out_act != ACT_NONE && a.out_act != ACT_RELU)) return 1;
  const bool two = a.split < c.rows;
  if (two && (!a.y2 || a.split < 0 || a.split % 16)) return 1;
  const int nblk = c.l16_J >= 16 ? 1 : 2;
  const int TC = 16 * nblk;
  const int gx = (n_max + TC - 1) / TC, gy = (c.rows + 15) / 16;
  if ((long long)gx * gy * B > o.env.lin16_max_tiles) return 1;
  const bool wide = c.K == 1 && c.l16_J == 6 && !ln && nblk == 2 && (gy % 4) == 0 && o.gate16_wide > 0 &&
                    (long long)gx * gy * B >= o.gate16_wide;
  if (!wide && c.K == 1 && B > 1 && !solo_tiles && (long long)gx * gy * B > 512) return 1;
  Lin16Args g;
  std::memset(&g, 0, sizeof(g));
  g.x = a.x; g.x_bs = a.x_bs; g.x_ld = a.x_ld;
  row_len(B, host_len, a.in_len, a.in_mul, a.in_const).into(g);
  g.len_mul = a.in_mul;
  g.w = arena + c.l16_w_off; g.bias = arena + c.l16_b_off; g.Cin = c.Cin; g.rows = c.rows; g.dil = a.dil; g.pad = a.pad;
  g.y = a.y; g.y_bs = a.y_bs; g.y_ld = a.y_ld; g.res = a.res; g.relu = a.out_act == ACT_RELU;
  g.split = two ? a.split : (1 << 30); g.y2 = a.y2; g.y2_bs = a.y2_bs; g.y2_ld = a.y2_ld; g.accum2 = a.accum2;
  const int shape = lin16_shape(c.K, c.l16_J, ln != nullptr, wide ? 4 : 1);
  if (shape < 0) return 1;
  if (ln) {
    g.ln_gamma = ln->gamma; g.ln_beta = ln->beta; g.ln_eps = 1e-4f; g.ln_relu = ln->relu; g.ln_out = ln->out;
  }
  ProfScope ps(ctx, w, cls, 2.0 * (double)c.Cout * c.Cin * c.K * (double)n_max * B);
  const dim3 grid(gx, wide ? gy / 4 : gy, B);
  switch_const<0, 1, 2, 3, 4, 5, 6, 7, 8>(shape, [&](auto i) {
    constexpr Lin16Shape t = LIN16_SHAPES[decltype(i)::value];
    hipLaunchKernelGGL(HIP_KERNEL_NAME(lin16_kernel<t.K, t.J, t.NBLK, t.LN, t.RTW>), grid, dim3(512), 0, w->stream, g);
  });
  ps.kernel(wide ? KN_LIN16_WIDE : ln ? KN_LIN16_LN : KN_LIN16);
  return 0;
}

static ConvArgs base_args(const float* x, long long x_bs, int x_ld, const int* in_len, int in_mul, float* y, long long y_bs,
                          int y_ld, const int* out_len, int out_mul, int dil, int pad) {
  ConvArgs a;
  std::memset(&a, 0, sizeof(a));
  a.x = x;
  a.x_bs = x_bs;
  a.x_ld = x_ld;
  a.in_len = in_len;
  a.in_mul = in_mul;
  a.y = y;
  a.y_bs = y_bs;
  a.y_ld = y_ld;
  a.out_len = out_len;
  a.out_mul = out_mul;
  a.dil = dil;
  a.pad = pad;
  a.in_slope = 1.0f;
  a.alpha = 1.0f;
  a.split = 1 << 30;
  a.out_act = ACT_NONE;
  return a;
}

static MelTransform to_mt(const mi355tts_audio_settings* s) {
  MelTransform m;
  std::memset(&m, 0, sizeof(m));
  if (!s) return m;
  m.signal_norm = s->signal_norm;
  m.symmetric_norm = s->symmetric_norm;
  m.clip_norm = s->clip_norm;
  m.convert_db_to_amp = s->convert_db_to_amp;
  m.do_drc = s->do_dynamic_range_compression;
  m.min_level_db = s->min_level_db;
  m.max_norm = s->max_norm;
  m.ref_level_db = s->ref_level_db;
  m.spec_gain = s->spec_gain;
  return m;
}
```

### larynx_amd/csrc/host_options.h

```cpp
#pragma once

constexpr int KNOB_UNSET = INT_MIN;
enum KnobWhen { PROCESS, CALL };
#define MI355TTS_ENV_KNOBS(X)                                                                                                       \
  X(sync_mode, "MI355TTS_SYNC_MODE", int, 3, PROCESS, "initial g_sync_mode: 0 hipStreamSynchronize, 1 blocking event, 2 query + sleep, 3 adaptive") \
  X(queue_policy, "MI355TTS_QUEUE_POLICY", int, 0, PROCESS, "acquire_worker: 1 = an idle hardware queue first, else the BUSIEST one (probe)") \
  X(queue_probe_off, "MI355TTS_NO_QUEUE_PROBE", bool, false, PROCESS, "no measurement of which worker streams share a hardware queue") \
  X(call_coalesce_off, "MI355TTS_NO_CALL_COALESCE", bool, false, PROCESS, "every call runs alone whatever option call_coalesce says") \
  X(selfcheck_off, "MI355TTS_NO_SELFCHECK", bool, false, PROCESS, "no dispatch-order self-check (looked at again when the check would run)") \
  X(rb_tiles, "MI355TTS_RB_TILES", int, 0, PROCESS, "workgroup target per ResBlock conv launch (<= 0: 1024)")                       \
  X(glow_tiles, "MI355TTS_GLOW_TILES", int, 0, PROCESS, "workgroup target per GlowTTS conv launch (<= 0: 1024)")                    \
  X(force_tile, "MI355TTS_FORCE_TILE", int, -1, PROCESS, "pins plan_conv's tile shape (0 .. 3): sweeps")                            \
  X(ups64, "MI355TTS_UPS64", bool, true, PROCESS, "64-row upsamplers on the 64 x 64 tile; 0 = plan_conv's shape rule (A/B runs)")   \
  X(m128_off, "MI355TTS_NO_M128", bool, false, PROCESS, "no 128-row tile at all")                                                    \
  X(m128_ups_off, "MI355TTS_NO_M128_UPS", bool, false, PROCESS, "no 128-row tile for the upsamplers")                                \
  X(rb_conv_off, "MI355TTS_NO_RB_CONV", bool, false, PROCESS, "grouped 128-row launches and upsamplers on the chunked tile, as option rb_conv = 0") \
  X(group_off, "MI355TTS_NO_GROUP", bool, false, PROCESS, "no grouped launches: neither run_group nor run_pair_group")               \
  X(group_promote_off, "MI355TTS_NO_GROUP_PROMOTE", bool, false, PROCESS, "batch-1 ResBlock steps stay on the tiles plan_conv chose") \
  X(snake_off, "MI355TTS_NO_SNAKE", bool, false, PROCESS, "grouped launches keep the longest-first order")                           \
  X(pair_fusion_off, "MI355TTS_NO_PAIR_FUSION", bool, false, PROCESS, "the 32 / 64-channel stages un-fused (every mode)")            \
  X(bf16_pair_off, "MI355TTS_NO_BF16_PAIR", bool, false, PROCESS, "the 32 / 64-channel stages un-fused in the bf16 modes")           \
  X(bf_k_off, "MI355TTS_NO_BF_K", bool, false, PROCESS, "no k-split tile in the bf16 modes")                                         \
  X(bf16_ups_off, "MI355TTS_NO_BF16_UPS", bool, false, PROCESS, "upsamplers stay f32 in the bf16 modes")                             \
  X(mrf8_off, "MI355TTS_NO_MRF8", bool, false, PROCESS, "the 8-channel stage on mrf_small_kernel instead of mrf8_kernel")            \
// ... 8 lines not shown
  X(att_big_lds, "MI355TTS_ATT_BIG_LDS", bool, false, PROCESS, "attention always on the P <= 768 instantiation (A/B runs)")         \
  X(wn_repeat, "MI355TTS_WN_REPEAT", int, 1, PROCESS, "wn_f16_kernel launched N times (probe: it is idempotent)")                   \
  X(force_tile_dynamic, "MI355TTS_FORCE_TILE_DYNAMIC", int, KNOB_UNSET, CALL, "as MI355TTS_FORCE_TILE and ahead of it (tests)")     \
  X(m128_min_tiles, "MI355TTS_M128_MIN_TILES", long long, 256, CALL, "workgroups a launch must yield before the 128-row tile is used (tests lower it)") \
  X(group_ncu, "MI355TTS_GROUP_NCU", int, KNOB_UNSET, CALL, "CUs the dispatch-order logic assumes (unset: the device's; tests)")    \
  X(promote_max_imbalance, "MI355TTS_PROMOTE_MAX_IMBALANCE", double, 1.35, CALL, "promote_group_plans: busiest CU / mean above which a step is not promoted") \
  X(rb_nb4_min_tiles, "MI355TTS_RB_NB4_MIN_TILES", int, KNOB_UNSET, CALL, "128-column ResBlock tiles from this many, whatever the load; 0 = never (unset: run_group's load rule)") \
  X(rb_pair_min_tiles, "MI355TTS_RB_PAIR_MIN_TILES", long long, 512, CALL, "tiles of the k = 11 member from which a fused step takes the 4-wave tile (tests lower it)") \
  X(bench_ablate, "MI355TTS_BENCH_ABLATE", int, 0, CALL, "mi355tts_bench_conv1d: ConvArgs::ablate (results are wrong when set)")

struct EnvKnobs {
#define X(field, name, type, def, when, doc) type field = def;
  MI355TTS_ENV_KNOBS(X)
#undef X
};
static void parse_knob(const char* e, bool* v) { *v = std::atoi(e) != 0; }
static void parse_knob(const char* e, int* v) { *v = std::atoi(e); }
static void parse_knob(const char* e, long long* v) { *v = std::atoll(e); }
static void parse_knob(const char* e, double* v) { *v = std::atof(e); }
static void read_env_knobs(KnobWhen which, EnvKnobs* k) {
#define X(field, name, type, def, when, doc)                          \
  if (when == which)                                                  \
    if (const char* e = std::getenv(name)) parse_knob(e, &k->field);
  MI355TTS_ENV_KNOBS(X)
#undef X
}
static EnvKnobs g_env;
static std::atomic<int> g_sync_mode{3};
static void init_process_knobs() {
  static const bool once = [] {
    read_env_knobs(PROCESS, &g_env);
    g_sync_mode.store(g_env.sync_mode, std::memory_order_relaxed);
    return true;
  }();
  (void)once;
}

#ifndef MI355TTS_CALL_COALESCE_DEFAULT
#define MI355TTS_CALL_COALESCE_DEFAULT 0
#endif

struct ContextOptions {
  std::atomic<bool> serial_branches{false};
  std::atomic<bool> adaptive_schedule{false};
  std::atomic<bool> gate16{true};
  std::atomic<int> gate16_wide{512};
  std::atomic<bool> glow_fuse{true};
  std::atomic<bool> voc_out{true};
  std::atomic<bool> mrf_small{true};
  std::atomic<bool> mrf_group{true};
  std::atomic<bool> rb_conv{true};
  std::atomic<bool> rb_pair{true};
  std::atomic<bool> rb_dil{true};
  std::atomic<bool> group_promote{true};
  std::atomic<bool> group_snake{true};
  std::atomic<int> call_coalesce{MI355TTS_CALL_COALESCE_DEFAULT};
  std::atomic<int> call_coalesce_window_us{300};
};

static const struct OptionRow {
  const char* name;
  std::atomic<bool> ContextOptions::*flag;
  std::atomic<int> ContextOptions::*count;
} option_table[] = {
    {"adaptive_schedule", &ContextOptions::adaptive_schedule, nullptr},
    {"mrf_small", &ContextOptions::mrf_small, nullptr},
    {"gate16", &ContextOptions::gate16, nullptr},
    {"call_coalesce", nullptr, &ContextOptions::call_coalesce},
    {"call_coalesce_window_us", nullptr, &ContextOptions::call_coalesce_window_us},
    {"glow_fuse", &ContextOptions::glow_fuse, nullptr},
    {"mrf_group", &ContextOptions::mrf_group, nullptr},
    {"rb_conv", &ContextOptions::rb_conv, nullptr},
    {"group_snake", &ContextOptions::group_snake, nullptr},
    {"group_promote", &ContextOptions::group_promote, nullptr},
    {"rb_pair", &ContextOptions::rb_pair, nullptr},
    {"rb_dil", &ContextOptions::rb_dil, nullptr},
    {"gate16_wide", nullptr, &ContextOptions::gate16_wide},
    {"voc_out", &ContextOptions::voc_out, nullptr},
    {"serial_branches", &ContextOptions::serial_branches, nullptr},
    {"sync_mode", nullptr, nullptr},
};
static int set_context_option(ContextOptions& c, const char* name, int value) {
  for (const OptionRow& r : option_table) {
    if (std::strcmp(name, r.name) != 0) continue;
    if (r.flag) {
      c.*r.flag = value != 0;
    } else if (r.count) {
      c.*r.count = value < 0 ? 0 : value;
    } else {
      if (value < 0 || value > 3) return fail(MI355TTS_ERR_INVALID, "sync_mode %d outside [0, 3]", value);
      g_sync_mode.store(value, std::memory_order_relaxed);
    }
    return 0;
  }
  return fail(MI355TTS_ERR_INVALID, "unknown option '%s'", name);
}

struct CallOptions {
  bool glow_fuse = true, gate16 = true, rb_conv = true, rb_pair = true, rb_dil = true, group_promote = true, group_snake = true;
  bool mrf_group = true, mrf_small = true, serial_branches = false, adaptive_schedule = false, voc_out = true;
  int gate16_wide = 512;
  int pin_tile = -1;
  int ncu = 256;
  EnvKnobs env;
};
static void snapshot_options(const ContextOptions& c, int device_ncu, CallOptions* o) {
  *o = CallOptions();
  o->env = g_env;
  read_env_knobs(CALL, &o->env);
  o->ncu = o->env.group_ncu != KNOB_UNSET ? o->env.group_ncu : device_ncu;
  o->glow_fuse = c.glow_fuse.load();
  o->gate16 = c.gate16.load();
  o->gate16_wide = c.gate16_wide.load();
  o->rb_conv = c.rb_conv.load();
  o->rb_pair = c.rb_pair.load();
  o->rb_dil = c.rb_dil.load();
  o->group_promote = c.group_promote.load();
  o->group_snake = c.group_snake.load();
  o->mrf_group = c.mrf_group.load();
  o->mrf_small = c.mrf_small.load();
  o->serial_branches = c.serial_branches.load();
  o->adaptive_schedule = c.adaptive_schedule.load();
  o->voc_out = c.voc_out.load();
}
```

### larynx_amd/csrc/mi355tts.hip

```cpp
#include <hip/hip_runtime.h>

#include <algorithm>
#include <time.h>
#include <sys/prctl.h>
#include <atomic>
#include <condition_variable>
#include <chrono>
#include <climits>
#include <cmath>
#include <cstdarg>
#include <cstdio>
#include <cstdlib>
#include <cstring>
#include <dlfcn.h>
#include <map>
#include <memory>
#include <mutex>
#include <string>
#include <utility>
#include <vector>

#include "../../include/mi355tts.h"
#include "conv_mfma.h"
#include "rb_conv.h"
// ... 655 lines not shown
extern "C" int mi355tts_op_conv1d(mi355tts_ctx* ctx, const float* x, int B, int Cin, int L, const int32_t* lens,
                                  const float* w, const float* bias, int Cout, int K, int dilation, float in_slope,
                                  int out_act, float* y) {
  return op_conv_common(ctx, x, B, Cin, L, lens, w, bias, Cout, K, dilation, in_slope, out_act, y, false);
}
extern "C" int mi355tts_op_conv_transpose1d(mi355tts_ctx* ctx, const float* x, int B, int Cin, int L, const float* w,
                                            const float* bias, int Cout, int K, int stride, float in_slope, float* y) {
  return op_conv_common(ctx, x, B, Cin, L, nullptr, w, bias, Cout, K, stride, in_slope, 0, y, true);
}

extern "C" int mi355tts_op_denoise(mi355tts_ctx* ctx, const float* wav, int B, int64_t N, const float* bias_spec,
                                   float strength, float* out) {
  if (!ctx || !wav || !bias_spec || !out || B <= 0 || N <= DN_FFT || (N % DN_HOP))
    return fail(MI355TTS_ERR_INVALID, "bad argument (N must be a multiple of 256 and > 1024)");
  CallFrame f(ctx);
  CHECK(f.open());
  Worker* w = f.w;
  hipStream_t s = f.s;
  const int T = (int)((N - DN_FFT + DN_HOP - 1) / DN_HOP);
  Carver cv;
  const size_t o_in = cv.take(sizeof(float) * (size_t)B * N);
  const size_t o_out = cv.take(sizeof(float) * (size_t)B * N);
  const size_t o_f = cv.take(sizeof(float) * (size_t)B * T * DN_FFT);
  const size_t o_b = cv.take(sizeof(float) * (DN_FFT / 2 + 1));
  const size_t o_fr = cv.take(sizeof(int) * B);
  CHECK(reserve(w, cv.pos));
  char* base = w->arena;
  float* din = (float*)(base + o_in);
  float* dout = (float*)(base + o_out);
  float* fb = (float*)(base + o_f);
  float* db = (float*)(base + o_b);
  int* dfr = (int*)(base + o_fr);
  std::vector<int> fr(B, (int)(N / DN_HOP));
  HIPCHECK(hipMemcpyAsync(din, wav, sizeof(float) * (size_t)B * N, hipMemcpyHostToDevice, s));
  HIPCHECK(hipMemcpyAsync(db, bias_spec, sizeof(float) * (DN_FFT / 2 + 1), hipMemcpyHostToDevice, s));
  HIPCHECK(hipMemcpyAsync(dfr, fr.data(), sizeof(int) * B, hipMemcpyHostToDevice, s));
  hipLaunchKernelGGL(stft_denoise_kernel, dim3(T, B), dim3(256), 0, s, din, (long long)N, dfr, DN_HOP, db, strength, fb, T,
                     (float*)nullptr);
  hipLaunchKernelGGL(overlap_add_kernel, dim3(256, B), dim3(256), 0, s, fb, T, dfr, DN_HOP, dout, (long long)N, (long long)N);
  HIPCHECK(hipMemcpyAsync(out, dout, sizeof(float) * (size_t)B * N, hipMemcpyDeviceToHost, s));
  return f.finish();
}

extern "C" int mi355tts_op_gauss_noise(mi355tts_ctx* ctx, uint64_t seed, int B, int C, int T, float* out) {
  if (!ctx || !out || B <= 0 || C <= 0 || T <= 0 || C > 65535 || B > 65535) return fail(MI355TTS_ERR_INVALID, "bad argument");
  CallFrame f(ctx);
  CHECK(f.open());
  const size_t n = (size_t)B * C * T;
  CHECK(reserve(f.w, n * sizeof(float)));
  float* d = (float*)f.w->arena;
  hipLaunchKernelGGL(noise_fill_kernel, dim3((T + 255) / 256, C, B), dim3(256), 0, f.s, d, C, T, seed);
  HIPCHECK(hipMemcpyAsync(out, d, n * sizeof(float), hipMemcpyDeviceToHost, f.s));
  return f.finish();
}

extern "C" int mi355tts_bench_conv1d(mi355tts_ctx* ctx, int B, int Cin, int Cout, int K, int dilation, int L,
                                     int tile_shape, int iters, float* ms_per_launch) {
  if (!ctx || !ms_per_launch || B <= 0 || Cin <= 0 || Cout <= 0 || L <= 0 || iters <= 0 || !(K % 2) || (L % 4))
    return fail(MI355TTS_ERR_INVALID, "bad argument (L must be a multiple of 4)");
  std::vector<float> wh((size_t)Cout * Cin * K), bh(Cout), xh((size_t)B * Cin * L);
  uint32_t st = 12345u;
  auto rnd = [&]() {
    st = st * 1664525u + 1013904223u;
    return ((st >> 8) * (1.0f / 16777216.0f)) * 2.0f - 1.0f;
  };
  const float sc = 1.0f / std::sqrt((float)Cin * K);
  for (auto& v : wh) v = rnd() * sc;
  for (auto& v : bh) v = rnd();
  for (auto& v : xh) v = rnd();
  ArenaBuilder ab;
  DevConv c = add_conv(ab, wh.data(), bh.data(), Cout, Cin, K, ROWS_PLAIN);
  CallFrame f(ctx);
  CHECK(f.open());
  Worker* w = f.w;
  hipStream_t s = f.s;
  Carver cv;
  const WorkerWeights ww(ab, cv);
  const size_t o_x = cv.take(sizeof(float) * xh.size());
  const size_t o_y = cv.take(sizeof(float) * (size_t)B * Cout * L);
  CHECK(reserve(w, cv.pos));
  char* base = w->arena;
  float* dx = (float*)(base + o_x);
  float* dy = (float*)(base + o_y);
  CHECK(ww.copy_and_bind(w, &c, 1));
  HIPCHECK(hipMemcpyAsync(dx, xh.data(), sizeof(float) * xh.size(), hipMemcpyHostToDevice, s));
  ConvArgs a = base_args(dx, (long long)Cin * L, L, nullptr, 1, dy, (long long)Cout * L, L, nullptr, 1, dilation,
                         (K * dilation - dilation) / 2);
  a.in_const = L;
  a.out_const = L;
  a.in_slope = 0.1f;
  a.ablate = w->opt.env.bench_ablate;
  const bool prof = ctx->profiling.load();
  ctx->profiling = false;
  w->opt.pin_tile = tile_shape;
  int rc = 0;
  for (int i = 0; i < 3 && !rc; ++i) rc = launch_conv(ctx, w, c, a, EPI_LINEAR, B, L, KC_RESBLOCK);
  hipEvent_t e0, e1;
  if (!rc && (hipEventCreate(&e0) != hipSuccess || hipEventCreate(&e1) != hipSuccess)) rc = fail(MI355TTS_ERR_HIP, "hipEventCreate");
  if (!rc) {
    hipEventRecord(e0, s);
    for (int i = 0; i < iters && !rc; ++i) rc = launch_conv(ctx, w, c, a, EPI_LINEAR, B, L, KC_RESBLOCK);
    hipEventRecord(e1, s);
    hipError_t e = f.wait();
    float ms = 0.f;
    if (e == hipSuccess) e = hipEventElapsedTime(&ms, e0, e1);
    if (e != hipSuccess) rc = fail(MI355TTS_ERR_HIP, "bench_conv1d: %s", hipGetErrorString(e));
// ... 161 lines not shown
```

### larynx_amd/csrc/rb_conv.h

```cpp
#pragma once
#include "conv_mfma.h"

namespace mi355tts {

#ifndef RB_STAMP
#define RB_STAMP(n)
#endif
#ifndef RB_PRIO
#define RB_PRIO 3
#endif
#ifndef RB_WIDE_STORES
#define RB_WIDE_STORES 1
#endif
#ifndef RB_ABL
#define RB_ABL 0
#endif

__device__ __forceinline__ int rb_opaque_off(int v) {
#if defined(__AMDGCN__)
  asm("" : "+v"(v));
#endif
  return v;
}
__device__ __forceinline__ float4 rb_a_load(const char* __restrict__ base, unsigned& lane_off) {
#if defined(__AMDGCN__)
  typedef float rb_f4 __attribute__((ext_vector_type(4)));
  unsigned long long p = reinterpret_cast<unsigned long long>(base);
  asm("" : "+s"(p), "+v"(lane_off));
  const rb_f4 v = *reinterpret_cast<const __attribute__((address_space(1))) rb_f4*>(p + lane_off);
  return make_float4(v.x, v.y, v.z, v.w);
#else
  return *reinterpret_cast<const float4*>(base + lane_off);
#endif
}

template <int HALO, int NB = 2, int CI_C = 16>
constexpr int rb_buf_floats() { return ((CI_C * (32 * NB + HALO) / 4 + 255) / 256) * 256 * 4; }
template <int HALO, int NB = 2, int CI_C = 16>
constexpr int rb_lds_floats() { return 4 * rb_buf_floats<HALO, NB, CI_C>(); }

template <int K, int HALO, int EPI = EPI_LINEAR, bool MRF = false, int NB = 2, int CI_C = 16, int DIL = 0>
__device__ __forceinline__ void rb_tile(const ConvArgs& a, const int tile_x, const int tile_y, const int b, float* __restrict__ xs) {
  static_assert(EPI == EPI_LINEAR || EPI == EPI_UPSAMPLE, "rb_tile: linear and upsample epilogues");
  constexpr int NT = 256, T_T = 32 * NB;
  constexpr int XW = T_T + HALO, XW4 = XW / 4, OCTS = CI_C / 8, S = OCTS * K;
  constexpr int NF4 = CI_C * XW4, NE = (NF4 + NT - 1) / NT;
  constexpr int BUF = rb_buf_floats<HALO, NB, CI_C>();
  static_assert(BUF == NE * NT * 4, "ring stride = whole thread sweeps");
  static_assert(XW % 4 == 0 && S >= NE + 2, "bad tile parameters");
  static_assert(DIL == 0 || ((K - 1) * DIL + (NB - 1) * 32 <= 255 && (K - 1) * DIL + 3 <= HALO), "tap offsets: ds_read2_b32 immediates, inside the halo");

  const int tid = threadIdx.x, lane = tid & 63, wm = tid >> 6;
  const int t0 = tile_x * T_T;
  const int mt0 = tile_y * 4 + wm;
  const int Lin = a.in_len ? a.in_len[b] * a.in_mul : a.in_const;
  const int Lout = a.out_len ? a.out_len[b] * a.out_mul : a.out_const;
  const int n_len = (EPI == EPI_UPSAMPLE) ? (Lin > 0 ? Lin + (K - 1) : 0) : Lout;
  if (t0 >= n_len) return;

  const float slope = a.in_slope;
  const float* xb = a.x + (long long)b * a.x_bs;
  const int nchunks = ((a.Cin + 7) / 8 + OCTS - 1) / OCTS;
  const int PA = (a.pad + 3) & ~3;
  const int used4 = (PA - a.pad + T_T + (K - 1) * a.dil + 3) >> 2;
  const int cin_last = a.Cin - 1, ld_last4 = a.x_ld - 4;

  constexpr int NP = MRF ? 3 : 1;
  const float* xb2 = MRF ? a.x2 + (long long)b * a.x_bs : nullptr;
  const float* xb3 = MRF ? a.x3 + (long long)b * a.x_bs : nullptr;
  float4 pre[NE * NP];
  auto gload = [&](int chunk) {
    const int cb = chunk * CI_C < cin_last ? chunk * CI_C : cin_last;
    const long long cbo = (long long)cb * a.x_ld;
#pragma unroll
    for (int i = 0; i < NE; ++i) {
      const int e = tid + NT * i;
      const int row = e / XW4, f = e - row * XW4;
      const int rowc = row < CI_C ? row : CI_C - 1, rel = rowc < cin_last - cb ? rowc : cin_last - cb;
      const int c0 = t0 - PA + 4 * f;
      const int off = rel * a.x_ld + (c0 < 0 ? 0 : (c0 > ld_last4 ? ld_last4 : c0));
      unsigned off4 = (unsigned)off * 4u;
      pre[i] = rb_a_load(reinterpret_cast<const char*>(xb + cbo), off4);
      if constexpr (MRF) {
        pre[NE + i] = rb_a_load(reinterpret_cast<const char*>(xb2 + cbo), off4);
        pre[2 * NE + i] = rb_a_load(reinterpret_cast<const char*>(xb3 + cbo), off4);
      }
    }
  };
  auto lstore1 = [&](int buf, int chunk, int i) {
    const int e = tid + NT * i;
    const int row = e / XW4, f = e - row * XW4;
    const int c0 = t0 - PA + 4 * f;
    const bool fok = row < a.Cin - chunk * CI_C && f < used4;
    float4 v = pre[i];
    if constexpr (MRF) {
      const float4 v2 = pre[NE + i], v3 = pre[2 * NE + i];
      v.x = ((v.x + v2.x) + v3.x) / a.in_div;
      v.y = ((v.y + v2.y) + v3.y) / a.in_div;
      v.z = ((v.z + v2.z) + v3.z) / a.in_div;
      v.w = ((v.w + v2.w) + v3.w) / a.in_div;
    }
    v.x = (fok && c0 >= 0 && c0 < Lin) ? v.x : 0.f;
    v.y = (fok && c0 + 1 >= 0 && c0 + 1 < Lin) ? v.y : 0.f;
    v.z = (fok && c0 + 2 >= 0 && c0 + 2 < Lin) ? v.z : 0.f;
    v.w = (fok && c0 + 3 >= 0 && c0 + 3 < Lin) ? v.w : 0.f;
    v.x = v.x > 0.f ? v.x : v.x * slope;
    v.y = v.y > 0.f ? v.y : v.y * slope;
    v.z = v.z > 0.f ? v.z : v.z * slope;
    v.w = v.w > 0.f ? v.w : v.w * slope;
    reinterpret_cast<float4*>(xs + buf * BUF)[e] = v;
  };

  floatx16 acc[NB];
#pragma unroll
  for (int nb = 0; nb < NB; ++nb)
#pragma unroll
    for (int r = 0; r < 16; ++r) acc[nb][r] = 0.f;

  const int mt0u = tile_y * 4 + __builtin_amdgcn_readfirstlane(wm);
  const char* wq = reinterpret_cast<const char*>(a.w) + (long long)mt0u * a.noct * K * 1024;
  unsigned lane16 = lane * 16;
  const int last_step = nchunks * S - 1;
  auto a_frag = [&](int chunk, int q) -> float4 {
    int g = chunk * S + q;
    g = g < last_step ? g : last_step;
    return rb_a_load(wq + (long long)g * 1024, lane16);
  };
  constexpr int RD = MI355TTS_ARING;
  float4 ar[RD];

  RB_STAMP(0);
  if (RB_PRIO) __builtin_amdgcn_s_setprio(RB_PRIO);
  gload(0);
#pragma unroll
  for (int i = 0; i < RD - 1; ++i) ar[i] = a_frag(0, i);
  {
    constexpr int NR = NE * NP;
    float4 p0[NR];
#pragma unroll
    for (int i = 0; i < NR; ++i) p0[i] = pre[i];
    gload(1);
    float4 p1[NR];
#pragma unroll
    for (int i = 0; i < NR; ++i) p1[i] = pre[i];
    gload(2);
    float4 p2[NR];
#pragma unroll
    for (int i = 0; i < NR; ++i) { p2[i] = pre[i]; pre[i] = p0[i]; }
#pragma unroll
    for (int i = 0; i < NE; ++i) lstore1(0, 0, i);
#pragma unroll
    for (int i = 0; i < NR; ++i) pre[i] = p1[i];
#pragma unroll
    for (int i = 0; i < NE; ++i) lstore1(1, 1, i);
#pragma unroll
    for (int i = 0; i < NR; ++i) pre[i] = p2[i];
  }
  __syncthreads();
  if (RB_PRIO) __builtin_amdgcn_s_setprio(0);
  RB_STAMP(1);

  const int b_off = (lane >> 5) * XW + (lane & 31) + (PA - a.pad);
// ... 102 lines not shown
          if (row0 >= a.rows) continue;
          const int co = row0 / a.up;
          const int n0 = q * a.up + (row0 - co * a.up) - a.up_pad;
          float* dst = a.y + (long long)b * a.y_bs + (long long)co * a.y_ld + n0;
          if (n0 >= 0 && n0 + 3 < Lout) {
            *reinterpret_cast<float4*>(dst) = make_float4(acc[nb][4 * g4] + bb[4 * g4], acc[nb][4 * g4 + 1] + bb[4 * g4 + 1],
                                                          acc[nb][4 * g4 + 2] + bb[4 * g4 + 2], acc[nb][4 * g4 + 3] + bb[4 * g4 + 3]);
          } else {
#pragma unroll
            for (int e = 0; e < 4; ++e)
              if (n0 + e >= 0 && n0 + e < Lout) dst[e] = acc[nb][4 * g4 + e] + bb[4 * g4 + e];
          }
        }
        continue;
      }
      if (a.up == 2) {
#pragma unroll
        for (int r = 0; r < 16; r += 2) {
          const int row = mt0 * 32 + (r & 3) + 8 * (r >> 2) + rbase;
          if (row >= a.rows) continue;
          const int co = row >> 1;
          const int n0 = q * 2 - a.up_pad;
          float* dst = a.y + (long long)b * a.y_bs + (long long)co * a.y_ld + n0;
          const float v0 = acc[nb][r] + bb[r], v1 = acc[nb][r + 1] + bb[r + 1];
          if (n0 >= 0 && n0 + 1 < Lout && row + 1 < a.rows) {
            typedef float up_float2 __attribute__((ext_vector_type(2), aligned(4)));
            *reinterpret_cast<up_float2*>(dst) = up_float2{v0, v1};
          } else {
            if (n0 >= 0 && n0 < Lout) dst[0] = v0;
            if (row + 1 < a.rows && n0 + 1 >= 0 && n0 + 1 < Lout) dst[1] = v1;
          }
        }
        continue;
      }
#pragma unroll
      for (int r = 0; r < 16; ++r) {
        const int row = mt0 * 32 + (r & 3) + 8 * (r >> 2) + rbase;
        if (row >= a.rows) continue;
        const int co = row / a.up;
        const int n = q * a.up + (row - co * a.up) - a.up_pad;
        if (n < 0 || n >= Lout) continue;
        a.y[(long long)b * a.y_bs + (long long)co * a.y_ld + n] = acc[nb][r] + bb[r];
      }
    }
  } else {
  const int col = lane & 31, rbase = 4 * (lane >> 5);
  const int row0 = mt0 * 32 + rbase;
  float* yb = a.y + (long long)b * a.y_bs;
  const float* rb = a.res ? a.res + (long long)b * a.y_bs : nullptr;
  const bool interior = tile_y * 128 + 128 <= a.rows && t0 + T_T <= Lout;
  float bb[16];
#pragma unroll
  for (int r = 0; r < 16; ++r) bb[r] = (RB_ABL & 16) ? 0.01f : a.bias[row0 + (r & 3) + 8 * (r >> 2)];
  if (interior && NB % 2 == 0 && RB_WIDE_STORES && (a.y_ld & 3) == 0) {
    __syncthreads();
    float* tw = xs + wm * (32 * 64);
    const int rbase0 = mt0 * 32;
#pragma unroll
    for (int np = 0; np < NB / 2; ++np) {
#pragma unroll
    for (int nb = 0; nb < 2; ++nb)
#pragma unroll
      for (int r = 0; r < 16; ++r) tw[((r & 3) + 8 * (r >> 2) + rbase) * 64 + nb * 32 + col] = acc[2 * np + nb][r] + bb[r];
    __builtin_amdgcn_wave_barrier();
#pragma unroll
    for (int h = 0; h < 2; ++h) {
      float4 v[4], rv[4];
      int off[4];
#pragma unroll
      for (int i = 0; i < 4; ++i) {
        const int idx = lane + 64 * (4 * h + i);
        const int row = idx >> 4, c4 = idx & 15;
        off[i] = (rbase0 + row) * a.y_ld + t0 + 64 * np + 4 * c4;
        v[i] = *reinterpret_cast<const float4*>(tw + row * 64 + 4 * c4);
      }
      if (rb && !(RB_ABL & 16)) {
#pragma unroll
        for (int i = 0; i < 4; ++i) rv[i] = *reinterpret_cast<const float4*>(rb + off[i]);
#pragma unroll
        for (int i = 0; i < 4; ++i) {
          v[i].x += rv[i].x;
          v[i].y += rv[i].y;
          v[i].z += rv[i].z;
          v[i].w += rv[i].w;
        }
      }
#pragma unroll
      for (int i = 0; i < 4; ++i) *reinterpret_cast<float4*>(yb + off[i]) = v[i];
    }
    if (np + 1 < NB / 2) __builtin_amdgcn_wave_barrier();
    }
  } else if (interior) {
    const int o0 = row0 * a.y_ld + t0 + col;
    if (rb && !(RB_ABL & 16)) {
#pragma unroll
      for (int nb = 0; nb < NB; ++nb) {
        float rv[16];
#pragma unroll
        for (int r = 0; r < 16; ++r) rv[r] = rb[o0 + ((r & 3) + 8 * (r >> 2)) * a.y_ld + nb * 32];
#pragma unroll
        for (int r = 0; r < 16; ++r) yb[o0 + ((r & 3) + 8 * (r >> 2)) * a.y_ld + nb * 32] = (acc[nb][r] + bb[r]) + rv[r];
      }
    } else {
#pragma unroll
      for (int nb = 0; nb < NB; ++nb)
#pragma unroll
        for (int r = 0; r < 16; ++r) yb[o0 + ((r & 3) + 8 * (r >> 2)) * a.y_ld + nb * 32] = acc[nb][r] + bb[r];
    }
  } else {
#pragma unroll
    for (int nb = 0; nb < NB; ++nb) {
      const int t = t0 + nb * 32 + col;
      const bool tok = t < Lout;
      const int tc = tok ? t : Lout - 1;
#pragma unroll
      for (int h = 0; h < 2; ++h) {
        float v[8];
        int off[8];
#pragma unroll
        for (int q = 0; q < 8; ++q) {
          const int r = 8 * h + q;
          const int row = row0 + (r & 3) + 8 * (r >> 2);
          off[q] = (row < a.rows ? row : a.rows - 1) * a.y_ld + tc;
          v[q] = acc[nb][r] + bb[r];
        }
        if (rb) {
          float rv[8];
#pragma unroll
          for (int q = 0; q < 8; ++q) rv[q] = rb[off[q]];
#pragma unroll
          for (int q = 0; q < 8; ++q) v[q] += rv[q];
        }
#pragma unroll
        for (int q = 0; q < 8; ++q) {
          const int r = 8 * h + q;
          if (tok && row0 + (r & 3) + 8 * (r >> 2) < a.rows) yb[off[q]] = v[q];
        }
      }
    }
  }
  }
  RB_STAMP(3);
}

template <int K, int HALO, int EPI, bool MRF, int CI_C = 16>
__global__ __launch_bounds__(256, CI_C == 16 ? 4 : 3) void rb_conv_kernel(const ConvArgs a) {
  __shared__ float xs[rb_lds_floats<HALO, 2, CI_C>()];
  int tile_x, tile_y;
  int gx = gridDim.x;
  const int lin = blockIdx.x + blockIdx.y * gridDim.x;
  if (gridDim.z > 1) {
    gx = row_tiles(conv_n_len<K, EPI>(a, blockIdx.z), 64);
    if (lin >= gx * (int)gridDim.y) return;
  }
  xcd_tile_lin(lin, gx, gridDim.y, tile_x, tile_y, a.rows_major);
  rb_tile<K, HALO, EPI, MRF, 2, CI_C>(a, tile_x, tile_y, blockIdx.z, xs);
}

template <int K> struct RbCfg;
template <> struct RbCfg<11> { static constexpr int HALO = 56; };
template <> struct RbCfg<7> { static constexpr int HALO = 36; };
template <> struct RbCfg<3> { static constexpr int HALO = 16; };

template <int K0, int K1, int K2, int NB, int DIL>
__device__ __forceinline__ void rb_group_body(const ConvGroupArgs& g, float* __restrict__ xs) {
  constexpr int H0 = RbCfg<K0>::HALO, H1 = RbCfg<K1>::HALO, H2 = RbCfg<K2>::HALO;
  const int lin = blockIdx.x;
  const int b = blockIdx.z;
  const bool ragged = gridDim.z > 1;
  int tx, ty;
  CONV_WG_STAMP(lin, 0);
  int m, l;
  if (g.nseg) {
    int sg = 0;
    while (sg + 1 < g.nseg && lin >= g.seg_off[sg + 1]) ++sg;
    m = g.seg_m[sg];
    l = g.seg_first[sg] + (lin - g.seg_off[sg]);
  } else {
    m = lin < g.off[1] ? 0 : lin < g.off[2] ? 1 : 2;
    l = lin - g.off[m];
  }
  if (m == 0) {
    const int gx = ragged ? row_tiles(conv_n_len<K0, EPI_LINEAR>(g.c[0], b), 32 * NB) : g.gx[0];
    if (l >= gx * g.gy[0]) return;
    xcd_tile_lin(l, gx, g.gy[0], tx, ty);
    rb_tile<K0, H0, EPI_LINEAR, false, NB, 16, DIL>(g.c[0], tx, ty, b, xs);
  } else if (m == 1) {
    const int gx = ragged ? row_tiles(conv_n_len<K1, EPI_LINEAR>(g.c[1], b), 32 * NB) : g.gx[1];
    if (l >= gx * g.gy[1]) return;
    xcd_tile_lin(l, gx, g.gy[1], tx, ty);
    rb_tile<K1, H1, EPI_LINEAR, false, NB, 16, DIL>(g.c[1], tx, ty, b, xs);
  } else {
    const int gx = ragged ? row_tiles(conv_n_len<K2, EPI_LINEAR>(g.c[2], b), 32 * NB) : g.gx[2];
    if (l >= gx * g.gy[2]) return;
    xcd_tile_lin(l, gx, g.gy[2], tx, ty);
    rb_tile<K2, H2, EPI_LINEAR, false, NB, 16, DIL>(g.c[2], tx, ty, b, xs);
  }
  CONV_WG_STAMP(lin, 1);
}
template <int K0, int K1, int K2, int NB>
constexpr int rb_group_lds_floats() {
  return max3(rb_lds_floats<RbCfg<K0>::HALO, NB>(), rb_lds_floats<RbCfg<K1>::HALO, NB>(), rb_lds_floats<RbCfg<K2>::HALO, NB>());
}

template <int K0, int K1, int K2, int NB = 2>
__global__ __launch_bounds__(256, NB > 2 ? 3 : 4) void rb_group_kernel(const ConvGroupArgs g) {
  __shared__ float xs[rb_group_lds_floats<K0, K1, K2, NB>()];
  rb_group_body<K0, K1, K2, NB, 0>(g, xs);
}
template <int K0, int K1, int K2, int NB, int DIL>
__global__ __launch_bounds__(256, NB > 2 ? 3 : 4) void rb_group_dil_kernel(const ConvGroupArgs g) {
  __shared__ float xs[rb_group_lds_floats<K0, K1, K2, NB>()];
  rb_group_body<K0, K1, K2, NB, DIL>(g, xs);
}

}
```

### larynx_amd/csrc/tile_grid.h

```cpp
#pragma once
#include <hip/hip_runtime.h>

#include <type_traits>

namespace mi355tts {

template <int V>
using int_c = std::integral_constant<int, V>;

constexpr int max3(int a, int b, int c) { return a > b ? (a > c ? a : c) : (b > c ? b : c); }

template <class B>
__device__ __forceinline__ int tile_len(const int* len, int mul, int len_const, B b) { return len ? len[b] * mul : len_const; }

__device__ __forceinline__ constexpr int acc_row(int r) { return (r & 3) + 8 * (r >> 2); }

__device__ __forceinline__ void xcd_tile_lin(int lin, int gx, int gy, int& tx, int& ty, int rows_major = 0) {
  const int n = gx * gy;
  const int xcd = lin & 7, slot = lin >> 3;
  const int q = n >> 3, r = n & 7;
  const int id = (xcd < r ? xcd * (q + 1) : r * (q + 1) + (xcd - r) * q) + slot;
  if (rows_major) {
    tx = id % gx;
    ty = id / gx;
  } else {
    ty = id % gy;
    tx = id / gy;
  }
}
__device__ __forceinline__ void xcd_tile(int gx, int gy, int& tx, int& ty, int rows_major = 0) {
  xcd_tile_lin(blockIdx.x + blockIdx.y * gx, gx, gy, tx, ty, rows_major);
}

__device__ __forceinline__ int row_tiles(int n_len, int tile) { return (n_len + tile - 1) / tile; }

}
```

### larynx_amd/csrc/voc_out.h

```cpp
#pragma once
#include <hip/hip_runtime.h>

#include "tile_grid.h"

namespace mi355tts {

constexpr int POST_TW = 256;
constexpr int POST_XW = POST_TW + 8;
constexpr int POST_CC = 16;

struct PostArgs {
  const float* x;
  const float* x2;
  const float* x3;
  float in_div, slope;
  long long x_bs;
  int x_ld;
  const int* len;
  int len_mul, len_const;
  const float* w;
  const float* bias;
  int C;
  float* y;
  long long y_bs;
  float* peak;
  long long peak_ld;
};

template <int K, int NPL>
__global__ __launch_bounds__(256) void post_conv_kernel(const PostArgs a) {
  static_assert(K == 7, "halo of 4 columns either side");
  __shared__ float xs[POST_CC * POST_XW];
  __shared__ float red[3 * POST_TW];
  const int tid = threadIdx.x;
  const int b = blockIdx.y;
  const int L = tile_len(a.len, a.len_mul, a.len_const, b);
  const int t0 = blockIdx.x * POST_TW;
  if (t0 >= L) return;
  const int i = tid & 63, h = tid >> 6;
  constexpr int XW4 = POST_XW / 4, NF4 = POST_CC * XW4, NE = (NF4 + 255) / 256;
  const float* xb[3] = {a.x + (long long)b * a.x_bs, (NPL > 1 ? a.x2 : a.x) + (long long)b * a.x_bs,
                        (NPL > 2 ? a.x3 : a.x) + (long long)b * a.x_bs};
  float4 pre[NPL][NE];
  auto request = [&](int c0) {
#pragma unroll
    for (int e = 0; e < NE; ++e) {
      const int f4 = tid + 256 * e;
      const int row = f4 / XW4 < POST_CC ? f4 / XW4 : POST_CC - 1, f = f4 - (f4 / XW4) * XW4;
      const int ch = c0 + row < a.C ? c0 + row : a.C - 1;
      const int col = t0 - 4 + 4 * f;
      const long long off = (long long)ch * a.x_ld + (col < 0 ? 0 : (col > a.x_ld - 4 ? a.x_ld - 4 : col));
#pragma unroll
      for (int p = 0; p < NPL; ++p) pre[p][e] = *reinterpret_cast<const float4*>(xb[p] + off);
    }
  };
  float acc[4] = {0.f, 0.f, 0.f, 0.f};
  request(0);
  for (int c0 = 0; c0 < a.C; c0 += POST_CC) {
    if (c0) __syncthreads();
#pragma unroll
    for (int e = 0; e < NE; ++e) {
      const int f4 = tid + 256 * e;
      const int row = f4 / XW4, f = f4 - row * XW4;
      const int col = t0 - 4 + 4 * f;
      const bool rok = c0 + row < a.C;
      float4 v = pre[0][e];
      if constexpr (NPL > 1) {
        v.x += pre[1][e].x;
        v.y += pre[1][e].y;
        v.z += pre[1][e].z;
        v.w += pre[1][e].w;
        if constexpr (NPL > 2) {
          v.x += pre[2][e].x;
          v.y += pre[2][e].y;
          v.z += pre[2][e].z;
          v.w += pre[2][e].w;
        }
        v.x = v.x / a.in_div;
        v.y = v.y / a.in_div;
        v.z = v.z / a.in_div;
        v.w = v.w / a.in_div;
      }
      v.x = (rok && col >= 0 && col < L) ? v.x : 0.f;
      v.y = (rok && col + 1 >= 0 && col + 1 < L) ? v.y : 0.f;
      v.z = (rok && col + 2 >= 0 && col + 2 < L) ? v.z : 0.f;
      v.w = (rok && col + 3 >= 0 && col + 3 < L) ? v.w : 0.f;
      v.x = v.x > 0.f ? v.x : v.x * a.slope;
      v.y = v.y > 0.f ? v.y : v.y * a.slope;
      v.z = v.z > 0.f ? v.z : v.z * a.slope;
      v.w = v.w > 0.f ? v.w : v.w * a.slope;
      if (f4 < NF4) reinterpret_cast<float4*>(xs)[f4] = v;
    }
    __syncthreads();
    request(c0 + POST_CC < a.C ? c0 + POST_CC : c0);
#pragma unroll
    for (int cc = 0; cc < POST_CC / 4; ++cc) {
      const int c = c0 + 4 * h + cc;
      const float4* xr = reinterpret_cast<const float4*>(xs + (4 * h + cc) * POST_XW) + i;
      const float4 p0 = xr[0], p1 = xr[1], p2 = xr[2];
      const float win[12] = {p0.x, p0.y, p0.z, p0.w, p1.x, p1.y, p1.z, p1.w, p2.x, p2.y, p2.z, p2.w};
      const float* wc = a.w + (c < a.C ? c : a.C - 1) * K;
      const float live = c < a.C ? 1.0f : 0.0f;
#pragma unroll
      for (int k = 0; k < K; ++k) {
        const float wk = wc[k] * live;
#pragma unroll
        for (int e = 0; e < 4; ++e) acc[e] = fmaf(wk, win[e + k + 1], acc[e]);
      }
    }
  }
  if (h > 0) *reinterpret_cast<float4*>(red + (h - 1) * POST_TW + 4 * i) = make_float4(acc[0], acc[1], acc[2], acc[3]);
  __syncthreads();
  float m = 0.f;
  if (h == 0) {
    const float bs = a.bias ? a.bias[0] : 0.f;
#pragma unroll
    for (int g = 0; g < 3; ++g) {
      const float4 o = *reinterpret_cast<const float4*>(red + g * POST_TW + 4 * i);
      acc[0] += o.x;
      acc[1] += o.y;
      acc[2] += o.z;
      acc[3] += o.w;
    }
    float4 v;
    v.x = tanhf(acc[0] + bs);
    v.y = tanhf(acc[1] + bs);
    v.z = tanhf(acc[2] + bs);
    v.w = tanhf(acc[3] + bs);
    const int t = t0 + 4 * i;
    float* yp = a.y + (long long)b * a.y_bs + t;
    if (t + 3 < L) {
      *reinterpret_cast<float4*>(yp) = v;
      m = fmaxf(fmaxf(fabsf(v.x), fabsf(v.y)), fmaxf(fabsf(v.z), fabsf(v.w)));
    } else {
      if (t < L) { yp[0] = v.x; m = fmaxf(m, fabsf(v.x)); }
      if (t + 1 < L) { yp[1] = v.y; m = fmaxf(m, fabsf(v.y)); }
      if (t + 2 < L) { yp[2] = v.z; m = fmaxf(m, fabsf(v.z)); }
    }
  }
  if (a.peak && h == 0) {
#pragma unroll
    for (int s = 32; s >= 1; s >>= 1) m = fmaxf(m, __shfl_xor(m, s));
    if (tid == 0) a.peak[(long long)b * a.peak_ld + blockIdx.x] = m;
  }
}

constexpr int VOC_MAX_ROWS = 16;

struct WaveOutArgs {
  const float* wav;
  long long bs;
  const int* frames;
  int hop;
  const float* peak;
  long long peak_ld;
  int peak_parts;
  float* f32;
  long long f_bs, f_ld;
  short* i16;
  long long i_bs, i_ld;
  int pad_before;
  int per_row;
  float* f32_rows[VOC_MAX_ROWS];
  short* i16_rows[VOC_MAX_ROWS];
  long long f_ld_rows[VOC_MAX_ROWS], i_ld_rows[VOC_MAX_ROWS];
  int pad_rows[VOC_MAX_ROWS];
};

__global__ __launch_bounds__(256) void wave_out_kernel(const WaveOutArgs a) {
  const int b = blockIdx.y;
  const long long N = (long long)a.frames[b] * a.hop;
  const float* src = a.wav + (long long)b * a.bs;
  const long long step = (long long)gridDim.x * blockDim.x, first = (long long)blockIdx.x * blockDim.x + threadIdx.x;
  const int pad_before = a.per_row ? a.pad_rows[b] : a.pad_before;
  float* const f32 = a.per_row ? a.f32_rows[b] : (a.f32 ? a.f32 + (long long)b * a.f_bs : nullptr);
  short* const i16 = a.per_row ? a.i16_rows[b] : (a.i16 ? a.i16 + (long long)b * a.i_bs : nullptr);
  if (f32) {
    float* dst = f32;
    const long long f_ld = a.per_row ? a.f_ld_rows[b] : a.f_ld;
    for (long long i = first; i < f_ld; i += step) {
      const long long j = i - pad_before;
      dst[i] = (j >= 0 && j < N) ? src[j] : 0.f;
    }
  }
  if (i16) {
    __shared__ float pm[4];
    const int np = a.peak_parts ? a.peak_parts : (int)((N + POST_TW - 1) / POST_TW);
    float m = 0.f;
    for (int i = threadIdx.x; i < np; i += blockDim.x) m = fmaxf(m, a.peak[(long long)b * a.peak_ld + i]);
#pragma unroll
    for (int sft = 32; sft >= 1; sft >>= 1) m = fmaxf(m, __shfl_xor(m, sft));
    if ((threadIdx.x & 63) == 0) pm[threadIdx.x >> 6] = m;
    __syncthreads();
    const float peak = fmaxf(0.01f, fmaxf(fmaxf(pm[0], pm[1]), fmaxf(pm[2], pm[3])));
    const float g = 32767.0f / peak;
    short* dst = i16;
    const long long i_ld = a.per_row ? a.i_ld_rows[b] : a.i_ld;
    for (long long i = first; i < i_ld; i += step) {
      short s = 0;
      const long long j = i - pad_before;
      if (j >= 0 && j < N) {
        float v = src[j] * g;
        v = fminf(fmaxf(v, -32767.0f), 32767.0f);
        s = (short)(int)v;
      }
      dst[i] = s;
    }
  }
}

}
```

### larynx_amd/engine.py

```python
from __future__ import annotations

import ctypes as C
import json
import threading
import typing
import weakref

import numpy as np

from . import ffi
from .hparams import GlowHParams, HifiGanHParams
from .weights import build_blob


class MelBatch:

    def __init__(self, engine: "Engine", handle: int, durations_ld: int = 0):
        self._engine = engine
        self._h = C.c_void_p(handle)
        self._durations: typing.Optional[np.ndarray] = None
        self._durations_ld = int(durations_ld)
        engine._live_mels.add(self)
        lib = engine.lib
        self.batch = ffi.check(lib, lib.mi355tts_mel_batch(self._h))
# ... 715 lines not shown
              want_f0: typing.Optional[int] = None) -> dict:
        audio, flat, B, N, n, f_in, i_in = self._audio_in(audio, samples)
        if not (want_float or want_int16):
            raise ValueError("nothing asked for: want_float and / or want_int16")
        ld = max([self.shift_length(model, int(v)) for v in n if 0 <= v <= N] or [0])
        f32 = np.empty((B, ld), np.float32) if want_float else None
        i16 = np.empty((B, ld), np.int16) if want_int16 else None
        pos = np.empty((B, int(want_positions)), np.int32) if want_positions is not None else None
        f0 = np.empty((B, int(want_f0)), np.float32) if want_f0 is not None else None
        pos_ld = int(want_positions or 0)
        if positions_in is not None:
            positions_in = np.ascontiguousarray(np.asarray(positions_in, np.int32).reshape(B, -1))
            pos_ld = positions_in.shape[1]
        out = self.shift_raw(model, f_in, i_in, n, N, ffi.ptr(f32), ffi.ptr(i16), ld, ffi.PCM_NORMALIZE if normalize else ffi.PCM_SATURATE,
                             positions_in_ptr=ffi.ptr(positions_in), positions_ptr=ffi.ptr(pos), pos_ld=pos_ld, f0_ptr=ffi.ptr(f0),
                             f0_ld=int(want_f0 or 0))
        f32, i16, pos, f0 = self._rows_out(flat, f32, i16, pos, f0)
        return {"f32": f32, "i16": i16, "samples": out, "positions": pos, "f0": f0}

    def shift_raw(self, model: int, f32_ptr, i16_ptr, samples, in_ld: int, out_f32_ptr, out_i16_ptr, out_ld: int, pcm_mode: int = 0,
                  positions_in_ptr=None, positions_ptr=None, pos_ld: int = 0, f0_ptr=None, f0_ld: int = 0, flags: int = 0) -> np.ndarray:
        n = np.ascontiguousarray(np.asarray(samples, np.int64).reshape(-1))
        out = np.zeros(len(n), np.int64)
        ffi.check(
            self.lib,
            self.lib.mi355tts_shift(self._ctx, int(model), f32_ptr, i16_ptr, n.ctypes.data_as(C.POINTER(C.c_int64)), len(n), int(in_ld),
                                    positions_in_ptr, out_f32_ptr, out_i16_ptr, int(out_ld), int(pcm_mode), positions_ptr, int(pos_ld),
                                    f0_ptr, int(f0_ld), out.ctypes.data_as(C.POINTER(C.c_int64)), int(flags)),
        )
        return out

    def conv1d(self, x, w, bias=None, dilation=1, in_slope=1.0, out_act=0, lens=None) -> np.ndarray:
        x = np.ascontiguousarray(x, np.float32)
        w = np.ascontiguousarray(w, np.float32)
        B, Cin, L = x.shape
        Cout, _, K = w.shape
        b = None if bias is None else np.ascontiguousarray(bias, np.float32)
        y = np.zeros((B, Cout, L), np.float32)
        ln = None if lens is None else np.ascontiguousarray(lens, np.int32)
        ffi.check(
            self.lib,
            self.lib.mi355tts_op_conv1d(
                self._ctx, x.ctypes.data, B, Cin, L, None if ln is None else ln.ctypes.data_as(C.POINTER(C.c_int32)),
                w.ctypes.data, ffi.ptr(b), Cout, K, int(dilation), float(in_slope), int(out_act), y.ctypes.data,
            ),
        )
        return y

    def gauss_noise(self, seed: int, B: int, channels: int, T: int) -> np.ndarray:
        out = np.empty((B, channels, T), np.float32)
        ffi.check(self.lib, self.lib.mi355tts_op_gauss_noise(self._ctx, int(seed) & (2 ** 64 - 1), B, channels, T, out.ctypes.data))
        return out

    def denoise(self, wav: np.ndarray, bias_spec: np.ndarray, strength: float) -> np.ndarray:
        wav = np.ascontiguousarray(wav, np.float32)
        if wav.ndim == 1:
            wav = wav[None]
        bias = np.ascontiguousarray(bias_spec, np.float32)
        out = np.zeros_like(wav)
        ffi.check(self.lib, self.lib.mi355tts_op_denoise(self._ctx, wav.ctypes.data, wav.shape[0], wav.shape[1], bias.ctypes.data,
                                                        float(strength), out.ctypes.data))
        return out

    def conv_transpose1d(self, x, w, bias, stride, in_slope=1.0) -> np.ndarray:
        x = np.ascontiguousarray(x, np.float32)
        w = np.ascontiguousarray(w, np.float32)
        B, Cin, L = x.shape
        _, Cout, K = w.shape
        b = None if bias is None else np.ascontiguousarray(bias, np.float32)
        y = np.zeros((B, Cout, L * stride), np.float32)
        ffi.check(
            self.lib,
            self.lib.mi355tts_op_conv_transpose1d(
                self._ctx, x.ctypes.data, B, Cin, L, w.ctypes.data, ffi.ptr(b), Cout, K, int(stride), float(in_slope), y.ctypes.data
            ),
        )
        return y

    def bench_conv1d(self, B, Cin, Cout, K, dilation, L, tile_shape=-1, iters=20) -> float:
        ms = C.c_float()
        ffi.check(self.lib, self.lib.mi355tts_bench_conv1d(self._ctx, B, Cin, Cout, K, dilation, L, tile_shape, iters, C.byref(ms)))
        return float(ms.value)

    def set_profiling(self, on: bool):
        ffi.check(self.lib, self.lib.mi355tts_set_profiling(self._ctx, 1 if on else 0))

    def set_option(self, name: str, value: int):
        ffi.check(self.lib, self.lib.mi355tts_set_option(self._ctx, name.encode("ascii"), int(value)))

    def coalesce_stats(self):
        a, b = C.c_int64(0), C.c_int64(0)
        ffi.check(self.lib, self.lib.mi355tts_coalesce_stats(self._ctx, C.byref(a), C.byref(b)))
        return int(a.value), int(b.value)

    def profile_reset(self):
        ffi.check(self.lib, self.lib.mi355tts_profile_reset(self._ctx))

    def profile_event_overhead_us(self, pairs: int = 64) -> float:
        us = C.c_double(0.0)
        ffi.check(self.lib, self.lib.mi355tts_profile_event_overhead(self._ctx, int(pairs), C.byref(us)))
        return float(us.value)

    def profile(self) -> dict:
        buf = C.create_string_buffer(4096)
        ffi.check(self.lib, self.lib.mi355tts_profile_json(self._ctx, buf, 4096))
        return json.loads(buf.value.decode("ascii"))
# ... 20 lines not shown
```

### larynx_amd/ffi.py

```python
from __future__ import annotations

import ctypes as C
import os
import threading
import typing
from pathlib import Path

import numpy as np

PACKAGE_DIR = Path(__file__).resolve().parent
DEFAULT_LIBRARY = PACKAGE_DIR / "libmi355tts.so"

MAX_STAGES = 8
IN_DEVICE = 1
OUT_DEVICE = 2
ABI_VERSION = 2
PRECISION_F32 = 0
PRECISION_BF16X3 = 1
PRECISION_BF16 = 2
PRECISION_F16 = 3
PRECISION_NOOP = 1


class GlowHParamsC(C.Structure):
# ... 155 lines not shown
    "mi355tts_load_analysis": (C.c_int, [_VP, C.POINTER(AnalysisParamsC), _VP, C.POINTER(C.c_int)]),
    "mi355tts_mel_from_audio": (
        C.c_int,
        [_VP, C.c_int, _VP, _VP, C.POINTER(C.c_int64), C.c_int, C.c_int64, C.POINTER(AudioSettingsC), C.c_uint32, C.POINTER(_VP)],
    ),
    "mi355tts_mel_plane": (C.c_int, [_VP, C.c_int, C.POINTER(_VP), C.POINTER(C.c_int)]),
    "mi355tts_load_resampler": (C.c_int, [_VP, C.POINTER(ResamplerParamsC), _VP, C.POINTER(C.c_int)]),
    "mi355tts_resample_length": (C.c_int64, [_VP, C.c_int, C.c_int64]),
    "mi355tts_resample": (
        C.c_int,
        [_VP, C.c_int, _VP, _VP, C.POINTER(C.c_int64), C.c_int, C.c_int64, _VP, _VP, C.c_int64, C.c_int, C.POINTER(C.c_int64), C.c_uint32],
    ),
    "mi355tts_load_loudness": (C.c_int, [_VP, C.POINTER(LoudnessParamsC), C.POINTER(C.c_int)]),
    "mi355tts_loudness": (
        C.c_int,
        [_VP, C.c_int, _VP, _VP, C.POINTER(C.c_int64), C.c_int, C.c_int64, C.c_float, C.c_float, C.c_float, _VP, _VP, C.c_int64,
         _VP, _VP, _VP, _VP, C.c_uint32],
    ),
    "mi355tts_load_limiter": (C.c_int, [_VP, C.POINTER(LimiterParamsC), _VP, _VP, C.POINTER(C.c_int)]),
    "mi355tts_limit": (
        C.c_int,
        [_VP, C.c_int, _VP, _VP, C.POINTER(C.c_int64), C.c_int, C.c_int64, _VP, C.c_float, _VP, _VP, C.c_int64, _VP, _VP, _VP, C.c_uint32],
    ),
    "mi355tts_load_pitch": (C.c_int, [_VP, C.POINTER(PitchParamsC), C.POINTER(C.c_int)]),
    "mi355tts_pitch_frames": (C.c_int64, [_VP, C.c_int, C.c_int64]),
    "mi355tts_pitch": (C.c_int, [_VP, C.c_int, _VP, _VP, C.POINTER(C.c_int64), C.c_int, C.c_int64, _VP, _VP, _VP, _VP, C.c_int64, C.c_uint32]),
    "mi355tts_load_shift": (C.c_int, [_VP, C.POINTER(ShiftParamsC), _VP, C.POINTER(C.c_int)]),
    "mi355tts_shift_length": (C.c_int64, [_VP, C.c_int, C.c_int64]),
    "mi355tts_shift": (
        C.c_int,
        [_VP, C.c_int, _VP, _VP, C.POINTER(C.c_int64), C.c_int, C.c_int64, _VP, _VP, _VP, C.c_int64, C.c_int, _VP, C.c_int64, _VP, C.c_int64,
         C.POINTER(C.c_int64), C.c_uint32],
    ),
    "mi355tts_synthesize": (
        C.c_int,
        [_VP, C.c_int, C.c_int, _VP, C.POINTER(C.c_int32), C.c_int, C.c_int, C.c_float, C.c_float, _VP, C.c_int, C.c_uint64,
         C.POINTER(AudioSettingsC), C.c_float, C.c_int32, C.c_int32, C.POINTER(C.c_int32), _VP, _VP, C.c_int64, C.c_uint32],
    ),
    "mi355tts_synthesize_speakers": (
        C.c_int,
        [_VP, C.c_int, C.c_int, _VP, C.POINTER(C.c_int32), C.c_int, C.c_int, C.c_float, C.c_float, _VP, C.c_int, C.c_uint64,
         C.POINTER(C.c_int32), C.POINTER(AudioSettingsC), C.c_float, C.c_int32, C.c_int32, C.POINTER(C.c_int32), _VP, _VP,
         C.c_int64, C.c_uint32],
    ),
    "mi355tts_synthesize_prosody": (
        C.c_int,
        [_VP, C.c_int, C.c_int, _VP, C.POINTER(C.c_int32), C.c_int, C.c_int, C.c_float, C.c_float, _VP, C.c_int, C.c_uint64,
         C.POINTER(C.c_int32), C.POINTER(AudioSettingsC), C.c_float, C.c_int32, C.c_int32, C.POINTER(C.c_int32), _VP, _VP,
         C.c_int64, C.c_uint32, C.POINTER(ProsodyC)],
    ),
    "mi355tts_reserve": (C.c_int, [_VP] + [C.c_int] * 8),
    "mi355tts_worker_queue_groups": (C.c_int, [_VP, C.POINTER(C.c_int32), C.c_int]),
    "mi355tts_op_gauss_noise": (C.c_int, [_VP, C.c_uint64, C.c_int, C.c_int, C.c_int, _VP]),
    "mi355tts_op_denoise": (C.c_int, [_VP, _VP, C.c_int, C.c_int64, _VP, C.c_float, _VP]),
    "mi355tts_op_conv1d": (
        C.c_int,
        [_VP, _VP, C.c_int, C.c_int, C.c_int, C.POINTER(C.c_int32), _VP, _VP, C.c_int, C.c_int, C.c_int, C.c_float, C.c_int, _VP],
    ),
    "mi355tts_op_conv_transpose1d": (
        C.c_int,
        [_VP, _VP, C.c_int, C.c_int, C.c_int, _VP, _VP, C.c_int, C.c_int, C.c_int, C.c_float, _VP],
    ),
    "mi355tts_hifigan_infer_taps": (C.c_int, [_VP, C.c_int, _VP, _VP, C.c_int64, C.c_char_p, C.c_int]),
    "mi355tts_voc_tap_copy": (C.c_int, [_VP, C.c_int, _VP, C.c_int64]),
    "mi355tts_bench_conv1d": (C.c_int, [_VP] + [C.c_int] * 8 + [C.POINTER(C.c_float)]),
    "mi355tts_set_profiling": (C.c_int, [_VP, C.c_int]),
    "mi355tts_set_option": (C.c_int, [_VP, C.c_char_p, C.c_int]),
    "mi355tts_coalesce_stats": (C.c_int, [_VP, C.POINTER(C.c_int64), C.POINTER(C.c_int64)]),
    "mi355tts_profile_reset": (C.c_int, [_VP]),
    "mi355tts_profile_json": (C.c_int, [_VP, C.c_char_p, C.c_int]),
    "mi355tts_call_coalesce_default": (C.c_int, []),
    "mi355tts_profile_kernels_json": (C.c_int, [_VP, C.c_char_p, C.c_int]),
    "mi355tts_kernel_counts_json": (C.c_int, [_VP, C.c_char_p, C.c_int]),
    "mi355tts_dispatch_selfcheck": (C.c_int, [_VP, C.POINTER(C.c_int), C.POINTER(C.c_float), C.POINTER(C.c_float)]),
    "mi355tts_profile_event_overhead": (C.c_int, [_VP, C.c_int, C.POINTER(C.c_double)]),
}

EXPORTED_SYMBOLS = tuple(sorted(_SIGNATURES))

_lib_lock = threading.Lock()
_libs: typing.Dict[str, C.CDLL] = {}


def load_library(path: typing.Union[str, os.PathLike, None] = None) -> C.CDLL:
    p = Path(path) if path is not None else DEFAULT_LIBRARY
    key = str(p.resolve())
    with _lib_lock:
        if key in _libs:
            return _libs[key]
        if not p.is_file():
            raise FileNotFoundError(
                f"{p} not found: the HIP library has not been built "
                "(run `python -m larynx_amd.build`; hipcc --offload-arch=gfx950 is required)"
            )
        lib = C.CDLL(key)
        for name, (res, args) in _SIGNATURES.items():
            fn = getattr(lib, name)
            fn.restype = res
            fn.argtypes = args
        ver = lib.mi355tts_abi_version()
        if ver != ABI_VERSION:
            raise RuntimeError(f"{p}: ABI version {ver}, expected {ABI_VERSION}")
        _libs[key] = lib
        return lib


# ... 68 lines not shown
```

Before: 303.4 utterances/s.

## Fuse leaky-ReLU into resblock conv epilogue and replace MRF divide with exact reciprocal

Adds a lean_staging option, on by default. The first resblock conv now applies leaky ReLU in its output epilogue, so the second conv reads already-activated data and skips the input activation. Dilation-1 groups with no activation use a plain kernel. The MRF average of three branches replaces the float division with a reciprocal multiply plus an FMA correction, intended to be bit-exact, and a device check op is added to verify that. Together these cut per-element ALU work in the vocoder staging, at the cost of more kernel variants and code complexity.

```diff
diff --git a/include/mi355tts.h b/include/mi355tts.h
--- a/include/mi355tts.h
+++ b/include/mi355tts.h
@@ -233,6 +233,9 @@
 
 int mi355tts_op_gauss_noise(mi355tts_ctx* ctx, uint64_t seed, int B, int C, int T, float* out);
 
+int mi355tts_op_mrf_average(mi355tts_ctx* ctx, const float* x, const float* x2, const float* x3, uint32_t first_bits, int64_t n, float div,
+                            float* out, uint64_t* mismatches);
+
 int mi355tts_op_maximum_path(mi355tts_ctx* ctx, const float* value, int B, int P_ld, int F_ld, const int32_t* id_lens,
                              const int32_t* frames, int32_t* durations_out, int dur_ld, float* score_out);
 
diff --git a/larynx_amd/csrc/conv_mfma.h b/larynx_amd/csrc/conv_mfma.h
--- a/larynx_amd/csrc/conv_mfma.h
+++ b/larynx_amd/csrc/conv_mfma.h
@@ -34,13 +34,14 @@
   EPI_UPSAMPLE = 3,
 };
 
-enum OutAct { ACT_NONE = 0, ACT_RELU = 1, ACT_TANH = 2 };
+enum OutAct { ACT_NONE = 0, ACT_RELU = 1, ACT_TANH = 2, ACT_LRELU = 3 };
 
 struct ConvArgs {
   const float* x;
   const float* x2;
   const float* x3;
   float in_div;
+  int in_div3;
   long long x_bs;
   int x_ld;
   const int* in_len;
@@ -54,6 +55,7 @@
   int dil;
   int pad;
   float in_slope;
+  float out_slope;
   float* y;
   long long y_bs;
   int y_ld;
@@ -103,7 +105,7 @@
   return XS > RED ? XS : RED;
 }
 
-template <int K, int CI_C, int MB, int NB, int WN, int KS, int HALO, int EPI, int WM = 1>
+template <int K, int CI_C, int MB, int NB, int WN, int KS, int HALO, int EPI, int WM = 1, bool DIV3 = false>
 __device__ __forceinline__ void conv_tile(const ConvArgs& a, const int tile_x, const int tile_y, const int b, float* __restrict__ xs) {
   static_assert(WM == 1 || EPI == EPI_LINEAR || EPI == EPI_UPSAMPLE, "row groups of waves: linear and upsample epilogues");
   constexpr int NWAVES = WM * WN * KS;
@@ -189,10 +191,10 @@
       }
 #pragma unroll
       for (int i = 0; i < NE; ++i) {
-        pre[i].x = pre[i].x / a.in_div;
-        pre[i].y = pre[i].y / a.in_div;
-        pre[i].z = pre[i].z / a.in_div;
-        pre[i].w = pre[i].w / a.in_div;
+        pre[i].x = mrf_avg<DIV3>(pre[i].x, a.in_div);
+        pre[i].y = mrf_avg<DIV3>(pre[i].y, a.in_div);
+        pre[i].z = mrf_avg<DIV3>(pre[i].z, a.in_div);
+        pre[i].w = mrf_avg<DIV3>(pre[i].w, a.in_div);
       }
     }
 #endif
@@ -441,7 +443,7 @@
       const float* rp = first ? a.res : nullptr;
       const bool acc_on = first ? (a.accum != 0) : (a.accum2 != 0);
       const float alpha = first ? a.alpha : 1.0f;
-      const int act = first ? a.out_act : (int)ACT_NONE;
+      const int act = first ? (a.out_slope != 1.0f ? (int)ACT_LRELU : a.out_act) : (int)ACT_NONE;
       float bb[R];
       int roff[R];
       bool rok[R];
@@ -501,6 +503,11 @@
         for (int nb = 0; nb < NB; ++nb)
 #pragma unroll
           for (int rr = 0; rr < R; ++rr) v[nb][rr] = tanhf(v[nb][rr]);
+      } else if (act == ACT_LRELU) {
+#pragma unroll
+        for (int nb = 0; nb < NB; ++nb)
+#pragma unroll
+          for (int rr = 0; rr < R; ++rr) v[nb][rr] = v[nb][rr] > 0.f ? v[nb][rr] : v[nb][rr] * a.out_slope;
       }
 #pragma unroll
       for (int nb = 0; nb < NB; ++nb)
@@ -680,7 +687,7 @@
 }
 
 
-template <int K, int CI_C, int MB, int NB, int WN, int KS, int HALO, int EPI, int WM = 1>
+template <int K, int CI_C, int MB, int NB, int WN, int KS, int HALO, int EPI, int WM = 1, bool DIV3 = false>
 __global__ __launch_bounds__(64 * WM * WN * KS, ((EPI == EPI_LINEAR && ((NB == 1 && MB == 2) || (MB == 1 && NB == 2 && KS == 4))) || WM == 4) ? 4 : 1) void conv_mfma_kernel(const ConvArgs a) {
   __shared__ float xs[conv_lds_floats<K, CI_C, MB, NB, WN, KS, HALO, EPI, WM>()];
   int tile_x, tile_y;
@@ -691,7 +698,7 @@
     if (lin >= gx * (int)gridDim.y) return;
   }
   xcd_tile_lin(lin, gx, gridDim.y, tile_x, tile_y, a.rows_major);
-  conv_tile<K, CI_C, MB, NB, WN, KS, HALO, EPI, WM>(a, tile_x, tile_y, blockIdx.z, xs);
+  conv_tile<K, CI_C, MB, NB, WN, KS, HALO, EPI, WM, DIV3>(a, tile_x, tile_y, blockIdx.z, xs);
   CONV_STAMP(5);
 }
 
diff --git a/larynx_amd/csrc/hifigan_forward.h b/larynx_amd/csrc/hifigan_forward.h
--- a/larynx_amd/csrc/hifigan_forward.h
+++ b/larynx_amd/csrc/hifigan_forward.h
@@ -166,12 +166,13 @@
   va_end(ap);
   return tmp;
 }
-static int voc_tap(VocPass& p, const std::string& name, const void* x, bool f16, int ch, int ld, int mul) {
+static int voc_tap(VocPass& p, const std::string& name, const void* x, bool f16, int ch, int ld, int mul, bool act = false) {
   VocTaps& T = *p.taps;
   VocTap t;
   t.name = name;
   t.kn = T.last_kn;
   t.f16 = f16;
+  t.act = act;
   t.B = p.B;
   t.ch = ch;
   t.ld = ld;
@@ -302,6 +303,7 @@
 static int f32_upsample(VocPass& p, const StageCursor<float>& c, const VocStage& st) {
   ConvArgs a = base_args(c.cur[0], (long long)c.ch * c.ldin, c.ldin, p.d_frames, c.mul, p.buf[1], st.bs, st.ldo, p.d_frames, st.mul, 1, st.ku / st.u - 1);
   c.inputs(a);
+  a.in_div3 = p.opt.lean_staging && a.x2 && a.in_div == 3.0f;
   a.in_slope = 0.1f;
   a.up = st.u;
   a.up_pad = (st.ku - st.u) / 2;
@@ -350,6 +352,7 @@
     }
   }
 
+  bool t_activated() const { return p.opt.lean_staging && p.prec == MI355TTS_PRECISION_F32; }
   int plan_step(int j, int d, VocStep& sp) const {
     const mi355tts_hifigan_hparams& h = p.hm->hp;
     const HifiResConv& rc = p.hm->rb[st.i][j][d];
@@ -366,11 +369,13 @@
       plan_pair(p.opt, rc.c1, rc.c2, x, sp.dst, bs, ldo, d_frames, mul, rc.dil, fold ? inv_nk : 1.0f, fold ? (j > 0) : 0, B, Lout, host_len,
                 &sp.pair, p.prec);
       if (sp.pair.ok) return 0;
+      const bool act_t = t_activated();
       ConvArgs a = base_args(x, bs, ldo, d_frames, mul, pl[j].t, bs, ldo, d_frames, mul, rc.dil, (kk * rc.dil - rc.dil) / 2);
       a.in_slope = 0.1f;
+      a.out_slope = act_t && !a.res ? 0.1f : 1.0f;
       CHECK(plan_conv(p.opt, rc.c1, a, EPI_LINEAR, B, Lout, KC_RESBLOCK, sc.rb_tiles, host_len, &sp.c1, p.prec));
       ConvArgs c2 = base_args(pl[j].t, bs, ldo, d_frames, mul, sp.dst, bs, ldo, d_frames, mul, 1, (kk - 1) / 2);
-      c2.in_slope = 0.1f;
+      c2.in_slope = act_t ? 1.0f : 0.1f;
       c2.res = x;
       if (fold) {
         c2.alpha = inv_nk;
@@ -392,7 +397,7 @@
   }
   int tap_step(int j, int d, const VocStep& sp) const {
     const bool fold = d == nd - 1 && !sc.split_out;
-    if (!sp.pair.ok && !sp.c2.empty) CHECK(voc_tap(p, tap_name("rb%d.%d.%d.t", st.i, j, d), pl[j].t, false, st.cout, st.ldo, st.mul));
+    if (!sp.pair.ok && !sp.c2.empty) CHECK(voc_tap(p, tap_name("rb%d.%d.%d.t", st.i, j, d), pl[j].t, false, st.cout, st.ldo, st.mul, t_activated()));
     if (!fold) return voc_tap(p, tap_name("rb%d.%d.%d", st.i, j, d), sp.dst, false, st.cout, st.ldo, st.mul);
     return j == nk - 1 ? voc_tap(p, tap_name("stage%d", st.i), sp.dst, false, st.cout, st.ldo, st.mul) : 0;
   }
@@ -488,6 +493,7 @@
     return 0;
   }
   PostArgs a = post_args<PostArgs>(p, c, (long long)c.ch * c.ldin);
+  a.in_div3 = p.opt.lean_staging && c.ncur > 1 && a.in_div == 3.0f;
   if (p.peak) {
     a.peak = p.peak;
     a.peak_ld = p.peak_ld;
@@ -496,7 +502,16 @@
     ProfScope ps(p.ctx, p.w, KC_VOC_IO, 2.0 * (double)c.ch * 7 * (double)c.Lin * p.B);
     ps.kernel(KN_POST_CONV);
     const dim3 pg((c.Lin + POST_TW - 1) / POST_TW, p.B);
-    switch_const<1, 2, 3>(c.ncur, [&](auto n) { hipLaunchKernelGGL(HIP_KERNEL_NAME(post_conv_kernel<7, decltype(n)::value>), pg, dim3(256), 0, p.s, a); });
+    switch_const<1, 2, 3>(c.ncur, [&](auto n) {
+      constexpr int NPL = decltype(n)::value;
+      if constexpr (NPL > 1) {
+        if (a.in_div3) {
+          hipLaunchKernelGGL(HIP_KERNEL_NAME(post_avg3_kernel<7, NPL>), pg, dim3(256), 0, p.s, a);
+          return;
+        }
+      }
+      hipLaunchKernelGGL(HIP_KERNEL_NAME(post_conv_kernel<7, NPL>), pg, dim3(256), 0, p.s, a);
+    });
   }
   if (p.taps) CHECK(voc_tap(p, "wav", p.wav, false, 1, (int)p.Nld, c.mul));
   return 0;
@@ -646,7 +661,7 @@
       if (p.taps) {
         const bool t_plane = h.resblock_type == 1 && pass == 0;
         for (int j = 0; j < nk; ++j)
-          CHECK(voc_tap(p, tap_name(t_plane ? "rb%d.%d.%d.t" : "rb%d.%d.%d", st.i, j, d), t_plane ? pl[j].t : dst[j], true, ch, st.ldo, st.mul));
+          CHECK(voc_tap(p, tap_name(t_plane ? "rb%d.%d.%d.t" : "rb%d.%d.%d", st.i, j, d), t_plane ? pl[j].t : dst[j], true, ch, st.ldo, st.mul, t_plane));
       }
     }
     for (int j = 0; j < nk; ++j) rin[j] = dst[j];
@@ -858,7 +873,7 @@
     std::snprintf(tmp, sizeof(tmp), "%s{\"name\": \"%s\", \"channels\": %d, \"ld\": %d, \"len\": [", i ? ", " : "", t.name.c_str(), t.ch, t.ld);
     s += tmp;
     for (size_t b = 0; b < t.len.size(); ++b) s += (b ? ", " : "") + std::to_string(t.len[b]);
-    std::snprintf(tmp, sizeof(tmp), "], \"f16\": %d, \"kernel\": \"%s\"}", t.f16 ? 1 : 0, t.kn >= 0 && t.kn < KN_COUNT ? kname_name[t.kn] : "-");
+    std::snprintf(tmp, sizeof(tmp), "], \"f16\": %d, \"act\": %d, \"kernel\": \"%s\"}", t.f16 ? 1 : 0, t.act ? 1 : 0, t.kn >= 0 && t.kn < KN_COUNT ? kname_name[t.kn] : "-");
     s += tmp;
   }
   return s + "]";
diff --git a/larynx_amd/csrc/host_context.h b/larynx_amd/csrc/host_context.h
--- a/larynx_amd/csrc/host_context.h
+++ b/larynx_amd/csrc/host_context.h
@@ -68,6 +68,7 @@
   std::string name;
   int kn = -1;
   bool f16 = false;
+  bool act = false;
   int B = 0, ch = 0, ld = 0;
   std::vector<int> len;
   void* dev = nullptr;
diff --git a/larynx_amd/csrc/host_launch.h b/larynx_amd/csrc/host_launch.h
--- a/larynx_amd/csrc/host_launch.h
+++ b/larynx_amd/csrc/host_launch.h
@@ -14,6 +14,12 @@
 template <int K, int CI_C, int MB, int NB, int WN, int KS, int HALO, int EPI>
 static void launch_conv_inst(ProfScope& ps, hipStream_t s, dim3 grid, const ConvArgs& a) {
   ps.kernel(KN_CONV_MFMA, a.rows);
+  if constexpr (EPI == EPI_UPSAMPLE) {
+    if (a.in_div3 && a.x2) {
+      hipLaunchKernelGGL(HIP_KERNEL_NAME(conv_mfma_kernel<K, CI_C, MB, NB, WN, KS, HALO, EPI, 1, true>), grid, dim3(64 * WN * KS), 0, s, a);
+      return;
+    }
+  }
   hipLaunchKernelGGL(HIP_KERNEL_NAME(conv_mfma_kernel<K, CI_C, MB, NB, WN, KS, HALO, EPI>), grid, dim3(64 * WN * KS), 0, s, a);
 }
 
@@ -40,7 +46,8 @@
     if (shape == TILE_M128) {
       if constexpr (K == 2) {
         if (rb_conv && a.Cin % 16 == 0 && !a.res && !a.accum && a.alpha == 1.0f && rb_plane_ok(a)) {
-          if (a.x2 && a.x3) hipLaunchKernelGGL(HIP_KERNEL_NAME(rb_conv_kernel<2, 4, EPI_UPSAMPLE, true>), grid, dim3(256), 0, s, a);
+          if (a.x2 && a.x3 && a.in_div3) hipLaunchKernelGGL(HIP_KERNEL_NAME(rb_conv_kernel<2, 4, EPI_UPSAMPLE, true, 16, true>), grid, dim3(256), 0, s, a);
+          else if (a.x2 && a.x3) hipLaunchKernelGGL(HIP_KERNEL_NAME(rb_conv_kernel<2, 4, EPI_UPSAMPLE, true>), grid, dim3(256), 0, s, a);
           else if (!a.x2) hipLaunchKernelGGL(HIP_KERNEL_NAME(rb_conv_kernel<2, 4, EPI_UPSAMPLE, false>), grid, dim3(256), 0, s, a);
           if ((a.x2 && a.x3) || !a.x2) {
             ps.kernel(KN_RB_CONV, a.rows);
@@ -49,7 +56,8 @@
         }
       }
       ps.kernel(KN_CONV_M128, a.rows);
-      hipLaunchKernelGGL(HIP_KERNEL_NAME(conv_mfma_kernel<K, 16, 1, 2, 1, 1, HALO, EPI, 4>), grid, dim3(256), 0, s, a);
+      if (a.in_div3 && a.x2) hipLaunchKernelGGL(HIP_KERNEL_NAME(conv_mfma_kernel<K, 16, 1, 2, 1, 1, HALO, EPI, 4, true>), grid, dim3(256), 0, s, a);
+      else hipLaunchKernelGGL(HIP_KERNEL_NAME(conv_mfma_kernel<K, 16, 1, 2, 1, 1, HALO, EPI, 4>), grid, dim3(256), 0, s, a);
       return 0;
     }
   }
@@ -288,7 +296,7 @@
 static bool rb_member_ok(const ConvArgs& a, int K) {
   const int halo = K == 11 ? RbCfg<11>::HALO : K == 7 ? RbCfg<7>::HALO : RbCfg<3>::HALO;
   return !a.x2 && !a.x3 && a.bias && a.alpha == 1.0f && !a.accum && a.out_act == ACT_NONE && a.split >= a.rows && !a.y2 &&
-         a.rows % 128 == 0 && halo_fits(K, a.dil, a.pad, halo) && rb_plane_ok(a);
+         (a.out_slope == 1.0f || !a.res) && a.rows % 128 == 0 && halo_fits(K, a.dil, a.pad, halo) && rb_plane_ok(a);
 }
 
 static void promote_group_plans(const CallOptions& o, ConvPlan* const* plans, int n) {
@@ -324,7 +332,11 @@
 }
 
 template <int NB>
-static void launch_rb_group(int dil, dim3 grid, hipStream_t s, const ConvGroupArgs& g) {
+static void launch_rb_group(int dil, bool act, dim3 grid, hipStream_t s, const ConvGroupArgs& g) {
+  if (dil == 1 && !act) {
+    hipLaunchKernelGGL(HIP_KERNEL_NAME(rb_group_plain_kernel<11, 7, 3, NB>), grid, dim3(256), 0, s, g);
+    return;
+  }
   const bool fixed = switch_const<1, 3, 5>(dil, [&](auto d) {
     hipLaunchKernelGGL(HIP_KERNEL_NAME(rb_group_dil_kernel<11, 7, 3, NB, decltype(d)::value>), grid, dim3(256), 0, s, g);
   });
@@ -381,6 +393,8 @@
     if (rb_ok) {
       const bool snake = o.group_snake && !o.env.snake_off;
       const int dil = (o.rb_dil && g.c[0].dil == g.c[1].dil && g.c[0].dil == g.c[2].dil) ? g.c[0].dil : 0;
+      bool act = !o.lean_staging;
+      for (int i = 0; i < 3; ++i) act = act || g.c[i].in_slope != 1.0f || g.c[i].out_slope != 1.0f;
       const int nb4_min = o.env.rb_nb4_min_tiles != KNOB_UNSET ? o.env.rb_nb4_min_tiles : (ctx->active_calls.load(std::memory_order_relaxed) > 1 ? 3 * ncu : 0);
       if (nb4_min > 0 && grid.z == 1) {
         int gx4[3], tiles4[3];
@@ -391,13 +405,13 @@
           const dim3 grid4(g.off[3], 1, 1);
           if (snake) group_snake_order(g, ncu, 3 * ncu);
           ps.kernel(KN_RB_GROUP_NB4, p0.a.rows);
-          launch_rb_group<4>(dil, grid4, s, g);
+          launch_rb_group<4>(dil, act, grid4, s, g);
           return 0;
         }
       }
       if (grid.z == 1 && snake) group_snake_order(g, ncu, 4 * ncu);
       ps.kernel(g.nseg ? KN_RB_GROUP_SNAKE : KN_RB_GROUP, p0.a.rows);
-      launch_rb_group<2>(dil, grid, s, g);
+      launch_rb_group<2>(dil, act, grid, s, g);
       return 0;
     }
   }
@@ -674,6 +688,7 @@
   a.dil = dil;
   a.pad = pad;
   a.in_slope = 1.0f;
+  a.out_slope = 1.0f;
   a.alpha = 1.0f;
   a.split = 1 << 30;
   a.out_act = ACT_NONE;
diff --git a/larynx_amd/csrc/host_options.h b/larynx_amd/csrc/host_options.h
--- a/larynx_amd/csrc/host_options.h
+++ b/larynx_amd/csrc/host_options.h
@@ -84,6 +84,7 @@
   std::atomic<bool> rb_conv{true};
   std::atomic<bool> rb_pair{true};
   std::atomic<bool> rb_dil{true};
+  std::atomic<bool> lean_staging{true};
   std::atomic<bool> group_promote{true};
   std::atomic<bool> group_snake{true};
   std::atomic<int> call_coalesce{MI355TTS_CALL_COALESCE_DEFAULT};
@@ -107,6 +108,7 @@
     {"group_promote", &ContextOptions::group_promote, nullptr},
     {"rb_pair", &ContextOptions::rb_pair, nullptr},
     {"rb_dil", &ContextOptions::rb_dil, nullptr},
+    {"lean_staging", &ContextOptions::lean_staging, nullptr},
     {"gate16_wide", nullptr, &ContextOptions::gate16_wide},
     {"voc_out", &ContextOptions::voc_out, nullptr},
     {"serial_branches", &ContextOptions::serial_branches, nullptr},
@@ -129,7 +131,7 @@
 }
 
 struct CallOptions {
-  bool glow_fuse = true, gate16 = true, rb_conv = true, rb_pair = true, rb_dil = true, group_promote = true, group_snake = true;
+  bool glow_fuse = true, gate16 = true, rb_conv = true, rb_pair = true, rb_dil = true, lean_staging = true, group_promote = true, group_snake = true;
   bool mrf_group = true, mrf_small = true, serial_branches = false, adaptive_schedule = false, voc_out = true;
   int gate16_wide = 512;
   int pin_tile = -1;
@@ -147,6 +149,7 @@
   o->rb_conv = c.rb_conv.load();
   o->rb_pair = c.rb_pair.load();
   o->rb_dil = c.rb_dil.load();
+  o->lean_staging = c.lean_staging.load();
   o->group_promote = c.group_promote.load();
   o->group_snake = c.group_snake.load();
   o->mrf_group = c.mrf_group.load();
diff --git a/larynx_amd/csrc/mi355tts.hip b/larynx_amd/csrc/mi355tts.hip
--- a/larynx_amd/csrc/mi355tts.hip
+++ b/larynx_amd/csrc/mi355tts.hip
@@ -731,6 +731,39 @@
   hipLaunchKernelGGL(noise_fill_kernel, dim3((T + 255) / 256, C, B), dim3(256), 0, f.s, d, C, T, seed);
   HIPCHECK(hipMemcpyAsync(out, d, n * sizeof(float), hipMemcpyDeviceToHost, f.s));
   return f.finish();
+}
+
+extern "C" int mi355tts_op_mrf_average(mi355tts_ctx* ctx, const float* x, const float* x2, const float* x3, uint32_t first_bits, int64_t n,
+                                       float div, float* out, uint64_t* mismatches) {
+  if (!ctx || !mismatches || n <= 0 || n > (1LL << 28) || (!x && (x2 || x3 || out))) return fail(MI355TTS_ERR_INVALID, "bad argument");
+  CallFrame f(ctx);
+  CHECK(f.open());
+  const bool host = x != nullptr;
+  const size_t plane = host ? sizeof(float) * (size_t)n : 0;
+  Carver cv;
+  const size_t o_c = cv.take(sizeof(unsigned));
+  const size_t o_x = cv.take(plane), o_x2 = cv.take(x2 ? plane : 0), o_x3 = cv.take(x3 ? plane : 0), o_y = cv.take(out ? plane : 0);
+  CHECK(reserve(f.w, cv.pos));
+  char* base = f.w->arena;
+  unsigned* dc = (unsigned*)(base + o_c);
+  HIPCHECK(hipMemsetAsync(dc, 0, sizeof(unsigned), f.s));
+  const float* planes[3] = {x, x2, x3};
+  const size_t offs[3] = {o_x, o_x2, o_x3};
+  const float* dp[3] = {nullptr, nullptr, nullptr};
+  for (int i = 0; i < 3; ++i)
+    if (planes[i]) {
+      dp[i] = (const float*)(base + offs[i]);
+      HIPCHECK(hipMemcpyAsync(base + offs[i], planes[i], plane, hipMemcpyHostToDevice, f.s));
+    }
+  float* dy = out ? (float*)(base + o_y) : nullptr;
+  const int blocks = (int)std::min<long long>((n + 255) / 256, 4096);
+  hipLaunchKernelGGL(mrf_avg_check_kernel, dim3(blocks), dim3(256), 0, f.s, dp[0], dp[1], dp[2], first_bits, (long long)n, div, dy, dc);
+  unsigned bad = 0;
+  HIPCHECK(hipMemcpyAsync(&bad, dc, sizeof(unsigned), hipMemcpyDeviceToHost, f.s));
+  if (out) HIPCHECK(hipMemcpyAsync(out, dy, plane, hipMemcpyDeviceToHost, f.s));
+  CHECK(f.finish());
+  *mismatches = bad;
+  return 0;
 }
 
 extern "C" int mi355tts_bench_conv1d(mi355tts_ctx* ctx, int B, int Cin, int Cout, int K, int dilation, int L,
diff --git a/larynx_amd/csrc/rb_conv.h b/larynx_amd/csrc/rb_conv.h
--- a/larynx_amd/csrc/rb_conv.h
+++ b/larynx_amd/csrc/rb_conv.h
@@ -39,7 +39,7 @@
 template <int HALO, int NB = 2, int CI_C = 16>
 constexpr int rb_lds_floats() { return 4 * rb_buf_floats<HALO, NB, CI_C>(); }
 
-template <int K, int HALO, int EPI = EPI_LINEAR, bool MRF = false, int NB = 2, int CI_C = 16, int DIL = 0>
+template <int K, int HALO, int EPI = EPI_LINEAR, bool MRF = false, int NB = 2, int CI_C = 16, int DIL = 0, bool ACT = true, bool DIV3 = false>
 __device__ __forceinline__ void rb_tile(const ConvArgs& a, const int tile_x, const int tile_y, const int b, float* __restrict__ xs) {
   static_assert(EPI == EPI_LINEAR || EPI == EPI_UPSAMPLE, "rb_tile: linear and upsample epilogues");
   constexpr int NT = 256, T_T = 32 * NB;
@@ -95,19 +95,21 @@
     float4 v = pre[i];
     if constexpr (MRF) {
       const float4 v2 = pre[NE + i], v3 = pre[2 * NE + i];
-      v.x = ((v.x + v2.x) + v3.x) / a.in_div;
-      v.y = ((v.y + v2.y) + v3.y) / a.in_div;
-      v.z = ((v.z + v2.z) + v3.z) / a.in_div;
-      v.w = ((v.w + v2.w) + v3.w) / a.in_div;
+      v.x = mrf_avg<DIV3>((v.x + v2.x) + v3.x, a.in_div);
+      v.y = mrf_avg<DIV3>((v.y + v2.y) + v3.y, a.in_div);
+      v.z = mrf_avg<DIV3>((v.z + v2.z) + v3.z, a.in_div);
+      v.w = mrf_avg<DIV3>((v.w + v2.w) + v3.w, a.in_div);
     }
     v.x = (fok && c0 >= 0 && c0 < Lin) ? v.x : 0.f;
     v.y = (fok && c0 + 1 >= 0 && c0 + 1 < Lin) ? v.y : 0.f;
     v.z = (fok && c0 + 2 >= 0 && c0 + 2 < Lin) ? v.z : 0.f;
     v.w = (fok && c0 + 3 >= 0 && c0 + 3 < Lin) ? v.w : 0.f;
-    v.x = v.x > 0.f ? v.x : v.x * slope;
-    v.y = v.y > 0.f ? v.y : v.y * slope;
-    v.z = v.z > 0.f ? v.z : v.z * slope;
-    v.w = v.w > 0.f ? v.w : v.w * slope;
+    if constexpr (ACT) {
+      v.x = v.x > 0.f ? v.x : v.x * slope;
+      v.y = v.y > 0.f ? v.y : v.y * slope;
+      v.z = v.z > 0.f ? v.z : v.z * slope;
+      v.w = v.w > 0.f ? v.w : v.w * slope;
+    }
     reinterpret_cast<float4*>(xs + buf * BUF)[e] = v;
   };
 
@@ -316,6 +318,20 @@
   float bb[16];
 #pragma unroll
   for (int r = 0; r < 16; ++r) bb[r] = (RB_ABL & 16) ? 0.01f : a.bias[row0 + (r & 3) + 8 * (r >> 2)];
+  if constexpr (ACT) {
+    if (a.out_slope != 1.0f && !rb) {
+      const float oslope = a.out_slope;
+#pragma unroll
+      for (int nb = 0; nb < NB; ++nb)
+#pragma unroll
+        for (int r = 0; r < 16; ++r) {
+          const float v = acc[nb][r] + bb[r];
+          acc[nb][r] = v > 0.f ? v : v * oslope;
+        }
+#pragma unroll
+      for (int r = 0; r < 16; ++r) bb[r] = -0.f;
+    }
+  }
   if (interior && NB % 2 == 0 && RB_WIDE_STORES && (a.y_ld & 3) == 0) {
     __syncthreads();
     float* tw = xs + wm * (32 * 64);
@@ -407,7 +423,7 @@
   RB_STAMP(3);
 }
 
-template <int K, int HALO, int EPI, bool MRF, int CI_C = 16>
+template <int K, int HALO, int EPI, bool MRF, int CI_C = 16, bool DIV3 = false>
 __global__ __launch_bounds__(256, CI_C == 16 ? 4 : 3) void rb_conv_kernel(const ConvArgs a) {
   __shared__ float xs[rb_lds_floats<HALO, 2, CI_C>()];
   int tile_x, tile_y;
@@ -418,7 +434,7 @@
     if (lin >= gx * (int)gridDim.y) return;
   }
   xcd_tile_lin(lin, gx, gridDim.y, tile_x, tile_y, a.rows_major);
-  rb_tile<K, HALO, EPI, MRF, 2, CI_C>(a, tile_x, tile_y, blockIdx.z, xs);
+  rb_tile<K, HALO, EPI, MRF, 2, CI_C, 0, true, DIV3>(a, tile_x, tile_y, blockIdx.z, xs);
 }
 
 template <int K> struct RbCfg;
@@ -426,7 +442,7 @@
 template <> struct RbCfg<7> { static constexpr int HALO = 36; };
 template <> struct RbCfg<3> { static constexpr int HALO = 16; };
 
-template <int K0, int K1, int K2, int NB, int DIL>
+template <int K0, int K1, int K2, int NB, int DIL, bool ACT = true>
 __device__ __forceinline__ void rb_group_body(const ConvGroupArgs& g, float* __restrict__ xs) {
   constexpr int H0 = RbCfg<K0>::HALO, H1 = RbCfg<K1>::HALO, H2 = RbCfg<K2>::HALO;
   const int lin = blockIdx.x;
@@ -448,17 +464,17 @@
     const int gx = ragged ? row_tiles(conv_n_len<K0, EPI_LINEAR>(g.c[0], b), 32 * NB) : g.gx[0];
     if (l >= gx * g.gy[0]) return;
     xcd_tile_lin(l, gx, g.gy[0], tx, ty);
-    rb_tile<K0, H0, EPI_LINEAR, false, NB, 16, DIL>(g.c[0], tx, ty, b, xs);
+    rb_tile<K0, H0, EPI_LINEAR, false, NB, 16, DIL, ACT>(g.c[0], tx, ty, b, xs);
   } else if (m == 1) {
     const int gx = ragged ? row_tiles(conv_n_len<K1, EPI_LINEAR>(g.c[1], b), 32 * NB) : g.gx[1];
     if (l >= gx * g.gy[1]) return;
     xcd_tile_lin(l, gx, g.gy[1], tx, ty);
-    rb_tile<K1, H1, EPI_LINEAR, false, NB, 16, DIL>(g.c[1], tx, ty, b, xs);
+    rb_tile<K1, H1, EPI_LINEAR, false, NB, 16, DIL, ACT>(g.c[1], tx, ty, b, xs);
   } else {
     const int gx = ragged ? row_tiles(conv_n_len<K2, EPI_LINEAR>(g.c[2], b), 32 * NB) : g.gx[2];
     if (l >= gx * g.gy[2]) return;
     xcd_tile_lin(l, gx, g.gy[2], tx, ty);
-    rb_tile<K2, H2, EPI_LINEAR, false, NB, 16, DIL>(g.c[2], tx, ty, b, xs);
+    rb_tile<K2, H2, EPI_LINEAR, false, NB, 16, DIL, ACT>(g.c[2], tx, ty, b, xs);
   }
   CONV_WG_STAMP(lin, 1);
 }
@@ -477,5 +493,10 @@
   __shared__ float xs[rb_group_lds_floats<K0, K1, K2, NB>()];
   rb_group_body<K0, K1, K2, NB, DIL>(g, xs);
 }
-
-}
+template <int K0, int K1, int K2, int NB>
+__global__ __launch_bounds__(256, NB > 2 ? 3 : 4) void rb_group_plain_kernel(const ConvGroupArgs g) {
+  __shared__ float xs[rb_group_lds_floats<K0, K1, K2, NB>()];
+  rb_group_body<K0, K1, K2, NB, 1, false>(g, xs);
+}
+
+}
diff --git a/larynx_amd/csrc/tile_grid.h b/larynx_amd/csrc/tile_grid.h
--- a/larynx_amd/csrc/tile_grid.h
+++ b/larynx_amd/csrc/tile_grid.h
@@ -14,6 +14,18 @@
 __device__ __forceinline__ int tile_len(const int* len, int mul, int len_const, B b) { return len ? len[b] * mul : len_const; }
 
 __device__ __forceinline__ constexpr int acc_row(int r) { return (r & 3) + 8 * (r >> 2); }
+
+template <bool DIV3>
+__device__ __forceinline__ float mrf_avg(float s, float div) {
+  if constexpr (DIV3) {
+    const float r = 1.0f / 3.0f;
+    const float q0 = s * r;
+    const float e = fmaf(-3.0f, q0, s);
+    return (e < 0.f || e > 0.f) ? fmaf(e, r, q0) : q0;
+  } else {
+    return s / div;
+  }
+}
 
 __device__ __forceinline__ void xcd_tile_lin(int lin, int gx, int gy, int& tx, int& ty, int rows_major = 0) {
   const int n = gx * gy;
diff --git a/larynx_amd/csrc/voc_out.h b/larynx_amd/csrc/voc_out.h
--- a/larynx_amd/csrc/voc_out.h
+++ b/larynx_amd/csrc/voc_out.h
@@ -14,6 +14,7 @@
   const float* x2;
   const float* x3;
   float in_div, slope;
+  int in_div3;
   long long x_bs;
   int x_ld;
   const int* len;
@@ -27,11 +28,9 @@
   long long peak_ld;
 };
 
-template <int K, int NPL>
-__global__ __launch_bounds__(256) void post_conv_kernel(const PostArgs a) {
+template <int K, int NPL, bool DIV3>
+__device__ __forceinline__ void post_conv_body(const PostArgs& a, float* __restrict__ xs, float* __restrict__ red) {
   static_assert(K == 7, "halo of 4 columns either side");
-  __shared__ float xs[POST_CC * POST_XW];
-  __shared__ float red[3 * POST_TW];
   const int tid = threadIdx.x;
   const int b = blockIdx.y;
   const int L = tile_len(a.len, a.len_mul, a.len_const, b);
@@ -76,10 +75,10 @@
           v.z += pre[2][e].z;
           v.w += pre[2][e].w;
         }
-        v.x = v.x / a.in_div;
-        v.y = v.y / a.in_div;
-        v.z = v.z / a.in_div;
-        v.w = v.w / a.in_div;
+        v.x = mrf_avg<DIV3>(v.x, a.in_div);
+        v.y = mrf_avg<DIV3>(v.y, a.in_div);
+        v.z = mrf_avg<DIV3>(v.z, a.in_div);
+        v.w = mrf_avg<DIV3>(v.w, a.in_div);
       }
       v.x = (rok && col >= 0 && col < L) ? v.x : 0.f;
       v.y = (rok && col + 1 >= 0 && col + 1 < L) ? v.y : 0.f;
@@ -143,6 +142,18 @@
     for (int s = 32; s >= 1; s >>= 1) m = fmaxf(m, __shfl_xor(m, s));
     if (tid == 0) a.peak[(long long)b * a.peak_ld + blockIdx.x] = m;
   }
+}
+template <int K, int NPL>
+__global__ __launch_bounds__(256) void post_conv_kernel(const PostArgs a) {
+  __shared__ float xs[POST_CC * POST_XW];
+  __shared__ float red[3 * POST_TW];
+  post_conv_body<K, NPL, false>(a, xs, red);
+}
+template <int K, int NPL>
+__global__ __launch_bounds__(256) void post_avg3_kernel(const PostArgs a) {
+  __shared__ float xs[POST_CC * POST_XW];
+  __shared__ float red[3 * POST_TW];
+  post_conv_body<K, NPL, true>(a, xs, red);
 }
 
 constexpr int VOC_MAX_ROWS = 16;
@@ -209,4 +220,18 @@
   }
 }
 
-}
+__global__ __launch_bounds__(256) void mrf_avg_check_kernel(const float* x, const float* x2, const float* x3, unsigned first, long long n, float div,
+                                                            float* out, unsigned* mismatches) {
+  unsigned bad = 0;
+  for (long long i = (long long)blockIdx.x * 256 + threadIdx.x; i < n; i += (long long)gridDim.x * 256) {
+    float s = x ? x[i] : __uint_as_float(first + (unsigned)i);
+    if (x2) s += x2[i];
+    if (x3) s += x3[i];
+    const float q = mrf_avg<true>(s, 3.0f), ref = mrf_avg<false>(s, div);
+    if (out) out[i] = q;
+    bad += __float_as_uint(q) != __float_as_uint(ref) ? 1u : 0u;
+  }
+  if (bad) atomicAdd(mismatches, bad);
+}
+
+}
diff --git a/larynx_amd/engine.py b/larynx_amd/engine.py
--- a/larynx_amd/engine.py
+++ b/larynx_amd/engine.py
@@ -791,6 +791,17 @@
         ffi.check(self.lib, self.lib.mi355tts_op_gauss_noise(self._ctx, int(seed) & (2 ** 64 - 1), B, channels, T, out.ctypes.data))
         return out
 
+    def mrf_average(self, x=None, x2=None, x3=None, first_bits: int = 0, n: int = 0, div: float = 3.0, want_out: bool = False):
+        planes = [None if a is None else np.ascontiguousarray(a, np.float32).ravel() for a in (x, x2, x3)]
+        if planes[0] is not None:
+            n = planes[0].size
+        out = np.empty(n, np.float32) if want_out and planes[0] is not None else None
+        bad = C.c_uint64()
+        ptrs = [None if a is None else a.ctypes.data for a in planes]
+        ffi.check(self.lib, self.lib.mi355tts_op_mrf_average(self._ctx, ptrs[0], ptrs[1], ptrs[2], int(first_bits) & 0xFFFFFFFF, int(n),
+                                                             float(div), None if out is None else out.ctypes.data, C.byref(bad)))
+        return int(bad.value), out
+
     def denoise(self, wav: np.ndarray, bias_spec: np.ndarray, strength: float) -> np.ndarray:
         wav = np.ascontiguousarray(wav, np.float32)
         if wav.ndim == 1:
diff --git a/larynx_amd/ffi.py b/larynx_amd/ffi.py
--- a/larynx_amd/ffi.py
+++ b/larynx_amd/ffi.py
@@ -231,6 +231,7 @@
     "mi355tts_reserve": (C.c_int, [_VP] + [C.c_int] * 8),
     "mi355tts_worker_queue_groups": (C.c_int, [_VP, C.POINTER(C.c_int32), C.c_int]),
     "mi355tts_op_gauss_noise": (C.c_int, [_VP, C.c_uint64, C.c_int, C.c_int, C.c_int, _VP]),
+    "mi355tts_op_mrf_average": (C.c_int, [_VP, _VP, _VP, _VP, C.c_uint32, C.c_int64, C.c_float, _VP, C.POINTER(C.c_uint64)]),
     "mi355tts_op_denoise": (C.c_int, [_VP, _VP, C.c_int, C.c_int64, _VP, C.c_float, _VP]),
     "mi355tts_op_conv1d": (
         C.c_int,
```

New measurement: 303.8 utterances/s (median of 4 runs). About the same (+0.1%).
